# tensorlayer/HyperPose

Hardware: NVIDIA H100
Metric: frames/sec end-to-end (conv+PAF parse) OpenPose-COCO 368x656 (higher is better)
Workload: dtype f16 operands, f32 accumulate (conv); f32/f64 (parse)

## Files before the change

hyperpose_b200/capi.py:

```python
from __future__ import annotations

import ctypes as C
import os
import struct

import numpy as np

PKG = os.path.dirname(os.path.abspath(__file__))
LIB_PATH = os.path.join(PKG, "libhyperpose_b200.so")

N_PARTS, N_PAIRS = 18, 19
HP_OK, HP_ERR_ARG, HP_ERR_CAPACITY, HP_ERR_UNSUPPORTED, HP_ERR_CUDA, HP_ERR_BATCH = 0, -1, -2, -3, -4, -5

PART_DT = np.dtype({"names": ["has_value", "x", "y", "score"], "formats": ["<i4", "<f4", "<f4", "<f4"]})
HUMAN_DT = np.dtype([("parts", PART_DT, (N_PARTS,)), ("score", "<f4")])
PEAK_DT = np.dtype([("part_id", "<i4"), ("x", "<i4"), ("y", "<i4"), ("score", "<f4"), ("id", "<i4")])
CONN_DT = np.dtype([("cid1", "<i4"), ("cid2", "<i4"), ("score", "<f4")])
assert HUMAN_DT.itemsize == 292

EXPORTS = [
    "hp_last_error", "hp_device_count", "hp_version",
    "hp_paf_create", "hp_paf_destroy", "hp_paf_set_conf_thresh", "hp_paf_set_paf_thresh", "hp_paf_set_capacity",
    "hp_paf_process_host", "hp_paf_process_host_batched", "hp_paf_process_device", "hp_paf_fetch",
    "hp_paf_debug_peaks", "hp_paf_debug_connections", "hp_paf_launch_count", "hp_paf_copy_results_device", "hp_paf_debug_timing",
# ... 83 lines not shown
        return out[:n.value].copy()

    def process_batch(self, conf: np.ndarray, paf: np.ndarray, cap: int = 128):
        conf = np.ascontiguousarray(conf, np.float32)
        paf = np.ascontiguousarray(paf, np.float32)
        N = conf.shape[0]
        out = np.zeros((N, cap), HUMAN_DT)
        n = (C.c_int * N)()
        check(lib().hp_paf_process_host_batched(self._h, conf.ctypes.data, paf.ctypes.data, N, conf.shape[1], paf.shape[1],
                                                conf.shape[2], conf.shape[3], out.ctypes.data, cap, n))
        return [out[i, :n[i]].copy() for i in range(N)]

    def process_device(self, d_conf_ptr: int, d_paf_ptr: int, N, c_conf, c_paf, H, W, stream: int = 0):
        check(lib().hp_paf_process_device(self._h, d_conf_ptr, d_paf_ptr, N, c_conf, c_paf, H, W, stream))

    def fetch(self, N: int, cap: int = 128):
        out = np.zeros((N, cap), HUMAN_DT)
        n = (C.c_int * N)()
        check(lib().hp_paf_fetch(self._h, out.ctypes.data, cap, n, N))
        return [out[i, :n[i]].copy() for i in range(N)]

    def debug_peaks(self, frame: int = 0, cap: int = 1 << 16) -> np.ndarray:
        out = np.zeros(cap, PEAK_DT)
        n = C.c_int(0)
        check(lib().hp_paf_debug_peaks(self._h, frame, out.ctypes.data, cap, C.byref(n)))
        return out[:n.value].copy()

    def debug_connections(self, frame: int, pair_id: int, cap: int = 4096) -> np.ndarray:
        out = np.zeros(cap, CONN_DT)
        n = C.c_int(0)
        check(lib().hp_paf_debug_connections(self._h, frame, pair_id, out.ctypes.data, cap, C.byref(n)))
        return out[:n.value].copy()

    @property
    def launch_count(self) -> int:
        return int(lib().hp_paf_launch_count(self._h))

    def debug_timing(self, N: int):
        out = np.zeros(N * (N_PAIRS * 4 + 6), np.uint64)
        lib().hp_paf_debug_timing.argtypes = [C.c_void_p, C.c_void_p, C.c_int]
        check(lib().hp_paf_debug_timing(self._h, out.ctypes.data, N))
        return out[:N * N_PAIRS * 4].reshape(N, N_PAIRS, 4), out[N * N_PAIRS * 4:].reshape(N, 6)

    PLAN_FIELDS = ("generic", "rz_mode", "tab_staged", "stage_bytes", "limb_dyn_bytes", "fast_asm", "wide_tile_rows", "wide_tile_cols")

    def debug_plan(self) -> dict:
        out = np.zeros(len(self.PLAN_FIELDS), np.int32)
        lib().hp_paf_debug_plan.argtypes = [C.c_void_p, C.c_void_p, C.c_int]
        check(lib().hp_paf_debug_plan(self._h, out.ctypes.data, len(out)))
        return dict(zip(self.PLAN_FIELDS, (int(v) for v in out)))

    def copy_results_device(self, d_humans_ptr: int, d_counts_ptr: int, N: int, cap: int, stream: int = 0):
        check(lib().hp_paf_copy_results_device(self._h, d_humans_ptr, d_counts_ptr, N, cap, stream))


def handoff_stats() -> dict:
    L = lib()
    if not getattr(L, "_engine_bound", False):
        _bind_engine(L)
        L._engine_bound = True
    v = [C.c_longlong() for _ in range(4)]
    check(L.hp_handoff_stats(*[C.byref(x) for x in v]))
    return dict(zip(("published", "hits", "batch_parses", "misses"), [x.value for x in v]))


def handoff_enable(on: bool):
    L = lib()
    if not getattr(L, "_engine_bound", False):
        _bind_engine(L)
        L._engine_bound = True
    check(L.hp_handoff_enable(1 if on else 0))


EXPORTS += [
    "hp_engine_create", "hp_engine_destroy", "hp_engine_info", "hp_engine_infer_u8_host", "hp_engine_infer_u8_device",
    "hp_engine_infer_f32_host", "hp_engine_outputs", "hp_engine_read_outputs_host", "hp_engine_copy_outputs_device", "hp_engine_sync",
    "hp_engine_launch_count", "hp_engine_debug_read_buffer", "hp_engine_debug_write_buffer", "hp_engine_debug_run_ops",
    "hp_pose_run_u8_host", "hp_engine_stage_frame_u8", "hp_engine_infer_staged", "hp_engine_debug_read_frames", "hp_engine_set_output_override", "hp_engine_set_profiling", "hp_engine_get_profile",
    "hp_engine_read_outputs_frames", "hp_engine_head_type", "hp_handoff_enable", "hp_handoff_stats",
    "hp_pose_submit_u8_host", "hp_pose_collect", "hp_pose_stats", "hp_paf_prepare", "hp_paf_state", "hp_paf_copy_results_host_async",
    "hp_paf_grow_capacity", "hp_pool_create", "hp_pool_destroy", "hp_pool_size", "hp_pool_set_capacity", "hp_pool_run_u8_host",
    "hp_pool_set_output_override", "hp_pool_launch_count", "hp_default_device", "hp_handoff_device_of",
    "hp_engine_create_ex", "hp_engine_dtype", "hp_pose_submit_u8_device", "hp_engine_debug_op_kernel",
    "hp_engine_debug_op_epilogue", "hp_engine_debug_op_conv_epilogue", "hp_engine_debug_uses_pdl",
    "hp_engine_debug_read_buffer_raw", "hp_engine_debug_write_outputs",
    "hp_engine_calibrate_u8", "hp_pack_int8_calibrated",
    "hp_pose_submit_frames_u8_host", "hp_pose_submit_frames_u8_device", "hp_pose_submit_pifpaf_frames_u8_host",
    "hp_pose_submit_pifpaf_frames_u8_device", "hp_pose_debug_read_slot_frames",
    "hp_pose_submit_frames_yuv420_host", "hp_pose_submit_frames_yuv420_device", "hp_pose_submit_pifpaf_frames_yuv420_host",
    "hp_pose_submit_pifpaf_frames_yuv420_device", "hp_pose_submit_ppn_frames_yuv420_host", "hp_pose_submit_ppn_frames_yuv420_device",
    "hp_pose_submit_frames_interleaved_host", "hp_pose_submit_frames_interleaved_device", "hp_pose_submit_pifpaf_frames_interleaved_host",
    "hp_pose_submit_pifpaf_frames_interleaved_device", "hp_pose_submit_ppn_frames_interleaved_host",
    "hp_pose_submit_ppn_frames_interleaved_device",
] + [f"hp_pose_submit{head}_frames_{fmt}_rotated_{where}" for head in ("", "_pifpaf", "_ppn") for fmt in ("yuv420", "interleaved")
     for where in ("host", "device")]


class FrameU8(C.Structure):
    _fields_ = [("data", C.c_void_p), ("height", C.c_int32), ("width", C.c_int32)]


class FrameYUV420(C.Structure):
    _fields_ = [("y", C.c_void_p), ("u", C.c_void_p), ("v", C.c_void_p), ("height", C.c_int32), ("width", C.c_int32),
                ("pitch_y", C.c_int32), ("pitch_uv", C.c_int32), ("uv_step", C.c_int32)]


YUV420_LAYOUTS = {"nv12": lambda H, W: (H * W, H * W + 1, W, 2), "nv21": lambda H, W: (H * W + 1, H * W, W, 2),
                  "i420": lambda H, W: (H * W, H * W + H * W // 4, W // 2, 1), "yv12": lambda H, W: (H * W + H * W // 4, H * W, W // 2, 1)}


def yuv420_record(frame: np.ndarray, layout: str) -> FrameYUV420:
    H, W = frame.shape[0] * 2 // 3, frame.shape[1]
    u, v, pitch_uv, step = YUV420_LAYOUTS[layout](H, W)
    p = frame.ctypes.data
    return FrameYUV420(p, p + u, p + v, H, W, W, pitch_uv, step)


class FrameInterleaved(C.Structure):
    _fields_ = [("data", C.c_void_p), ("height", C.c_int32), ("width", C.c_int32), ("pitch", C.c_int32), ("format", C.c_int32)]


PIXEL_FORMATS = {"bgr": 0, "rgb": 1, "bgra": 2, "rgba": 3, "gray": 4, "yuyv": 5, "uyvy": 6, "yvyu": 7}
PIXEL_CHANNELS = {"bgr": 3, "rgb": 3, "bgra": 4, "rgba": 4, "gray": None, "yuyv": 2, "uyvy": 2, "yvyu": 2}


def interleaved_record(frame: np.ndarray, fmt: str) -> FrameInterleaved:
    return FrameInterleaved(frame.ctypes.data, frame.shape[0], frame.shape[1], frame.strides[0], PIXEL_FORMATS[fmt])


ROTATIONS = (0, 90, 180, 270)


def rotation_table(rotation, n: int):
    rots = None
    if isinstance(rotation, (int, np.integer)):
        rots = [rotation] * n
    elif isinstance(rotation, (list, tuple, np.ndarray)):
        rots = list(rotation)
    if rots is None or len(rots) != n:
        raise HyperposeError(HP_ERR_ARG, f"rotation {rotation!r}: expected one of {ROTATIONS} degrees, or one per frame ({n})")
    for i, r in enumerate(rots):
        if isinstance(r, (bool, np.bool_)) or not isinstance(r, (int, np.integer)) or int(r) not in ROTATIONS:
            raise HyperposeError(HP_ERR_ARG, f"frame {i}: rotation {r!r} is not one of {ROTATIONS} clockwise degrees")
    return (C.c_int32 * n)(*[int(r) for r in rots])


def _bind_engine(L):
    vp, ip = C.c_void_p, C.POINTER(C.c_int)
    L.hp_engine_create.argtypes = [C.POINTER(vp), vp, C.c_size_t, C.c_int, C.c_int, C.c_int, C.c_double, C.c_int, C.c_int]
    L.hp_engine_create_ex.argtypes = [C.POINTER(vp), vp, C.c_size_t, C.c_int, C.c_int, C.c_int, C.c_double, C.c_int, C.c_int, C.c_int]
    L.hp_engine_dtype.argtypes = [vp]
    L.hp_engine_destroy.argtypes = [vp]
    L.hp_engine_destroy.restype = None
    L.hp_engine_info.argtypes = [vp, ip, ip, ip, ip, ip, ip, ip, C.POINTER(C.c_double)]
    L.hp_engine_infer_u8_host.argtypes = [vp, vp, C.c_int]
    L.hp_engine_infer_u8_device.argtypes = [vp, vp, C.c_int, vp]
    L.hp_engine_infer_f32_host.argtypes = [vp, vp, C.c_int]
    L.hp_engine_outputs.argtypes = [vp, C.POINTER(vp), C.POINTER(vp), C.POINTER(vp)]
    L.hp_engine_read_outputs_host.argtypes = [vp, vp, vp, C.c_int]
    L.hp_engine_sync.argtypes = [vp]
    L.hp_engine_copy_outputs_device.argtypes = [vp, vp, vp, C.c_int, vp]
    L.hp_engine_launch_count.argtypes = [vp]
    L.hp_engine_launch_count.restype = C.c_longlong
    L.hp_engine_debug_read_buffer.argtypes = [vp, C.c_int, vp, C.c_int, ip, ip, ip]
    L.hp_engine_debug_write_buffer.argtypes = [vp, C.c_int, vp, C.c_int]
    L.hp_engine_debug_run_ops.argtypes = [vp, C.c_int, C.c_int, C.c_int]
    L.hp_engine_debug_op_kernel.argtypes = [vp, C.c_int, C.c_char_p, C.c_int]
    L.hp_engine_debug_op_epilogue.argtypes = [vp, C.c_int, ip]
    L.hp_engine_debug_op_conv_epilogue.argtypes = [vp, C.c_int, ip]
    L.hp_engine_debug_uses_pdl.argtypes = [vp, ip]
    L.hp_engine_debug_read_buffer_raw.argtypes = [vp, C.c_int, vp, C.c_int]
    L.hp_engine_debug_write_outputs.argtypes = [vp, vp, vp, C.c_int]
    L.hp_engine_calibrate_u8.argtypes = [vp, vp, C.c_int, vp, C.c_int]
    L.hp_pack_int8_calibrated.argtypes = [vp, C.c_size_t]
    L.hp_pose_run_u8_host.argtypes = [vp, vp, vp, C.c_int, vp, C.c_int, ip]
    L.hp_engine_stage_frame_u8.argtypes = [vp, C.c_int, vp, C.c_int, C.c_int, C.c_int]
    L.hp_engine_infer_staged.argtypes = [vp, C.c_int]
    L.hp_engine_debug_read_frames.argtypes = [vp, vp, C.c_int]
    L.hp_engine_set_output_override.argtypes = [vp, vp, vp]
    L.hp_engine_set_profiling.argtypes = [vp, C.c_int]
    L.hp_engine_get_profile.argtypes = [vp, vp, vp, vp, C.c_int, ip, C.POINTER(C.c_longlong)]
    L.hp_engine_read_outputs_frames.argtypes = [vp, C.POINTER(vp), C.POINTER(vp), C.c_int, C.c_int]
    L.hp_engine_head_type.argtypes = [vp]
    L.hp_handoff_enable.argtypes = [C.c_int]
    L.hp_handoff_stats.argtypes = [C.POINTER(C.c_longlong)] * 4
    L.hp_pose_submit_u8_host.argtypes = [vp, vp, vp, C.c_int, ip]
    L.hp_pose_submit_u8_device.argtypes = [vp, vp, vp, C.c_int, ip]
    L.hp_pose_collect.argtypes = [vp, C.c_int, vp, C.c_int, ip]
    for f in (L.hp_pose_submit_frames_u8_host, L.hp_pose_submit_frames_u8_device, L.hp_pose_submit_pifpaf_frames_u8_host,
              L.hp_pose_submit_pifpaf_frames_u8_device, L.hp_pose_submit_ppn_frames_u8_host, L.hp_pose_submit_ppn_frames_u8_device):
        f.argtypes = [vp, vp, C.POINTER(FrameU8), C.c_int, C.c_int, ip]
    for f in (L.hp_pose_submit_frames_yuv420_host, L.hp_pose_submit_frames_yuv420_device, L.hp_pose_submit_pifpaf_frames_yuv420_host,
              L.hp_pose_submit_pifpaf_frames_yuv420_device, L.hp_pose_submit_ppn_frames_yuv420_host, L.hp_pose_submit_ppn_frames_yuv420_device):
        f.argtypes = [vp, vp, C.POINTER(FrameYUV420), C.c_int, C.c_int, ip]
    for f in (L.hp_pose_submit_frames_interleaved_host, L.hp_pose_submit_frames_interleaved_device,
              L.hp_pose_submit_pifpaf_frames_interleaved_host, L.hp_pose_submit_pifpaf_frames_interleaved_device,
              L.hp_pose_submit_ppn_frames_interleaved_host, L.hp_pose_submit_ppn_frames_interleaved_device):
        f.argtypes = [vp, vp, C.POINTER(FrameInterleaved), C.c_int, C.c_int, ip]
    for head in ("", "_pifpaf", "_ppn"):
        for fmt, rec in (("yuv420", FrameYUV420), ("interleaved", FrameInterleaved)):
            for where in ("host", "device"):
                getattr(L, f"hp_pose_submit{head}_frames_{fmt}_rotated_{where}").argtypes = \
                    [vp, vp, C.POINTER(rec), C.POINTER(C.c_int32), C.c_int, C.c_int, ip]
    L.hp_pose_submit_ppn_u8_host.argtypes = [vp, vp, vp, C.c_int, ip]
    L.hp_pose_submit_ppn_u8_device.argtypes = [vp, vp, vp, C.c_int, ip]
    L.hp_pose_debug_read_slot_frames.argtypes = [vp, C.c_int, vp, C.c_int]
    L.hp_pose_stats.argtypes = [vp, C.POINTER(C.c_longlong), C.POINTER(C.c_longlong)]
    L.hp_pool_create.argtypes = [C.POINTER(vp), ip, C.c_int, vp, C.c_size_t, C.c_int, C.c_int, C.c_int, C.c_double, C.c_int, C.c_float, C.c_float]
    L.hp_pool_destroy.argtypes = [vp]
    L.hp_pool_destroy.restype = None
    L.hp_pool_size.argtypes = [vp]
    L.hp_pool_set_capacity.argtypes = [vp, C.c_int, C.c_int, C.c_int]
    L.hp_pool_run_u8_host.argtypes = [vp, vp, C.c_int, vp, C.c_int, ip]
    L.hp_pool_set_output_override.argtypes = [vp, C.POINTER(vp), C.POINTER(vp)]
    L.hp_pool_launch_count.argtypes = [vp]
    L.hp_pool_launch_count.restype = C.c_longlong
    L.hp_default_device.restype = C.c_int
    L.hp_handoff_device_of.argtypes = [vp]


class Engine:

    def __init__(self, pack: bytes, input_size, max_batch_size: int = 8, factor: float = 1.0 / 255, flip_rgb: bool = True,
                 device: int = 0, dtype: str = "f16"):
        L = lib()
        if not getattr(L, "_engine_bound", False):
            _bind_engine(L)
            L._engine_bound = True
        self._h = C.c_void_p()
        self._pack = pack
        self.dtype = dtype
        check(L.hp_engine_create_ex(C.byref(self._h), pack, len(pack), int(input_size[0]), int(input_size[1]), max_batch_size,
                                    factor, 1 if flip_rgb else 0, device, {"f16": 0, "tf32": 1, "int8": 2}[dtype]))
        v = [C.c_int() for _ in range(7)]
        fl = C.c_double()
        check(L.hp_engine_info(self._h, *[C.byref(x) for x in v], C.byref(fl)))
        (self.in_w, self.in_h, self.max_batch, self.c_conf, self.c_paf, self.out_h, self.out_w) = [x.value for x in v]
        self.flops_per_frame = fl.value

    def close(self):
        if getattr(self, "_h", None) and _lib is not None:
            _lib.hp_engine_destroy(self._h)
        self._h = None

    def __del__(self):
        try:
            self.close()
        except Exception:
            pass

    def max_batch_size(self):
        return self.max_batch
# ... 42 lines not shown
        return conf, paf

    def read_outputs_frames(self, n: int, publish: bool = False):
        if self.head_type == 1:
            sa, sb = (17, 5, self.out_h, self.out_w), (19, 9, self.out_h, self.out_w)
        else:
            sa, sb = (self.c_conf, self.out_h, self.out_w), (self.c_paf, self.out_h, self.out_w)
        a = [np.empty(sa, np.float32) for _ in range(n)]
        b = [np.empty(sb, np.float32) for _ in range(n)]
        pa = (C.c_void_p * n)(*[x.ctypes.data for x in a])
        pb = (C.c_void_p * n)(*[x.ctypes.data for x in b])
        check(lib().hp_engine_read_outputs_frames(self._h, pa, pb, n, 1 if publish else 0))
        return [[a[i], b[i]] for i in range(n)]

    @property
    def head_type(self) -> int:
        return int(lib().hp_engine_head_type(self._h))

    def device_outputs(self):
        a, b, s = C.c_void_p(), C.c_void_p(), C.c_void_p()
        check(lib().hp_engine_outputs(self._h, C.byref(a), C.byref(b), C.byref(s)))
        return a.value, b.value, (s.value or 0)

    def sync(self):
        check(lib().hp_engine_sync(self._h))

    def copy_outputs_device(self, d_conf_ptr: int, d_paf_ptr: int, n: int, stream: int = 0):
        check(lib().hp_engine_copy_outputs_device(self._h, d_conf_ptr, d_paf_ptr, n, stream))

    @property
    def launch_count(self) -> int:
        return int(lib().hp_engine_launch_count(self._h))

    def debug_read_buffer(self, buf: int, n: int, raw: bool = False) -> np.ndarray:
        H, W, Cc = C.c_int(), C.c_int(), C.c_int()
        check(lib().hp_engine_debug_read_buffer(self._h, buf, None, n, C.byref(H), C.byref(W), C.byref(Cc)))
        out = np.empty((n, H.value, W.value, Cc.value), self._elem)
        if raw:
            check(lib().hp_engine_debug_read_buffer_raw(self._h, buf, out.ctypes.data, n))
        else:
            check(lib().hp_engine_debug_read_buffer(self._h, buf, out.ctypes.data, n, C.byref(H), C.byref(W), C.byref(Cc)))
        return out

    def debug_write_outputs(self, conf: np.ndarray, paf: np.ndarray):
        conf, paf = np.ascontiguousarray(conf, np.float32), np.ascontiguousarray(paf, np.float32)
        assert conf.shape[0] == paf.shape[0]
        assert conf.shape[1:] == (self.c_conf, self.out_h, self.out_w) and paf.shape[1:] == (self.c_paf, self.out_h, self.out_w)
        check(lib().hp_engine_debug_write_outputs(self._h, conf.ctypes.data, paf.ctypes.data, conf.shape[0]))

    def debug_write_buffer(self, buf: int, arr: np.ndarray):
        arr = np.ascontiguousarray(arr, self._elem)
        check(lib().hp_engine_debug_write_buffer(self._h, buf, arr.ctypes.data, arr.shape[0]))

    @property
    def _elem(self):
        return {"f16": np.float16, "tf32": np.float32, "int8": np.int8}[self.dtype]

    def calibrate(self, frames: np.ndarray, absmax=None) -> np.ndarray:
        frames = np.ascontiguousarray(frames, np.uint8)
        assert frames.ndim == 4 and frames.shape[1:] == (self.in_h, self.in_w, 3), frames.shape
        n_buf = struct.unpack_from("<I", self._pack, 12)[0]
        out = np.zeros(n_buf, np.float32) if absmax is None else np.array(absmax, np.float32).reshape(-1).copy()
        check(lib().hp_engine_calibrate_u8(self._h, frames.ctypes.data, frames.shape[0], out.ctypes.data, out.size))
        return out

    def debug_run_ops(self, first: int, last: int, n: int):
        check(lib().hp_engine_debug_run_ops(self._h, first, last, n))

    def debug_op_kernel(self, op: int) -> str:
        buf = C.create_string_buffer(64)
        check(lib().hp_engine_debug_op_kernel(self._h, op, buf, len(buf)))
        return buf.value.decode()

    def debug_op_epilogue(self, op: int) -> str:
        v = C.c_int(0)
        check(lib().hp_engine_debug_op_epilogue(self._h, op, C.byref(v)))
        return "tma" if v.value else "reg"

    def debug_op_conv_epilogue(self, op: int) -> str:
        v = C.c_int(0)
        check(lib().hp_engine_debug_op_conv_epilogue(self._h, op, C.byref(v)))
        return "tma" if v.value else "reg"

    def debug_uses_pdl(self) -> bool:
        v = C.c_int(0)
        check(lib().hp_engine_debug_uses_pdl(self._h, C.byref(v)))
        return bool(v.value)

    def set_output_override(self, d_conf_ptr: int, d_paf_ptr: int):
        check(lib().hp_engine_set_output_override(self._h, d_conf_ptr, d_paf_ptr))

    def set_profiling(self, enable: bool):
        check(lib().hp_engine_set_profiling(self._h, 1 if enable else 0))

    def get_profile(self):
        cap = 1024
        ms = np.zeros(cap, np.float64); ty = np.zeros(cap, np.int32); fl = np.zeros(cap, np.float64)
        n, runs = C.c_int(), C.c_longlong()
        check(lib().hp_engine_get_profile(self._h, ms.ctypes.data, ty.ctypes.data, fl.ctypes.data, cap, C.byref(n), C.byref(runs)))
        return ms[:n.value], ty[:n.value], fl[:n.value], runs.value

    def run_pose(self, parser: "PafParser", frames: np.ndarray, cap: int = 128):
        frames = np.ascontiguousarray(frames, np.uint8)
        N = frames.shape[0]
        out = np.zeros((N, cap), HUMAN_DT)
        n = (C.c_int * N)()
        check(lib().hp_pose_run_u8_host(self._h, parser._h, frames.ctypes.data, N, out.ctypes.data, cap, n))
        return [out[i, :n[i]].copy() for i in range(N)]


    def submit_pose(self, parser: "PafParser", frames: np.ndarray) -> int:
        assert frames.dtype == np.uint8 and frames.flags["C_CONTIGUOUS"]
        t = C.c_int(-1)
        if isinstance(parser, PifPafParser):
            lib().hp_pose_submit_pifpaf_u8_host.argtypes = [C.c_void_p, C.c_void_p, C.c_void_p, C.c_int, C.POINTER(C.c_int)]
            check(lib().hp_pose_submit_pifpaf_u8_host(self._h, parser._h, frames.ctypes.data, frames.shape[0], C.byref(t)))
        elif isinstance(parser, PoseProposalParser):
            check(lib().hp_pose_submit_ppn_u8_host(self._h, parser._h, frames.ctypes.data, frames.shape[0], C.byref(t)))
        else:
            check(lib().hp_pose_submit_u8_host(self._h, parser._h, frames.ctypes.data, frames.shape[0], C.byref(t)))
        self._ticket_n = getattr(self, "_ticket_n", {})
        self._ticket_n[t.value] = frames.shape[0]
        return t.value

    def submit_pose_device(self, parser: "PafParser", d_frames_ptr: int, n: int) -> int:
        t = C.c_int(-1)
        if isinstance(parser, PifPafParser):
            lib().hp_pose_submit_pifpaf_u8_device.argtypes = [C.c_void_p, C.c_void_p, C.c_void_p, C.c_int, C.POINTER(C.c_int)]
            check(lib().hp_pose_submit_pifpaf_u8_device(self._h, parser._h, d_frames_ptr, n, C.byref(t)))
        elif isinstance(parser, PoseProposalParser):
            check(lib().hp_pose_submit_ppn_u8_device(self._h, parser._h, d_frames_ptr, n, C.byref(t)))
        else:
            check(lib().hp_pose_submit_u8_device(self._h, parser._h, d_frames_ptr, n, C.byref(t)))
        self._ticket_n = getattr(self, "_ticket_n", {})
        self._ticket_n[t.value] = n
        return t.value

    def _submit_frame_table(self, parser, table, keep_ratio, device: bool, fmt: str = "u8", rotation=None) -> int:
        t = C.c_int(-1)
        head = "_pifpaf" if isinstance(parser, PifPafParser) else "_ppn" if isinstance(parser, PoseProposalParser) else ""
        where = "device" if device else "host"
        if rotation is None:
            fn = getattr(lib(), f"hp_pose_submit{head}_frames_{fmt}_{where}")
            check(fn(self._h, parser._h, table, len(table), 1 if keep_ratio else 0, C.byref(t)))
        else:
            fn = getattr(lib(), f"hp_pose_submit{head}_frames_{fmt}_rotated_{where}")
            check(fn(self._h, parser._h, table, rotation, len(table), 1 if keep_ratio else 0, C.byref(t)))
        self._ticket_n = getattr(self, "_ticket_n", {})
        self._ticket_n[t.value] = len(table)
        return t.value

    def submit_pose_frames(self, parser, frames, keep_ratio: bool = False) -> int:
        for i, f in enumerate(frames):
            if not isinstance(f, np.ndarray) or f.dtype != np.uint8 or f.ndim != 3 or f.shape[2] != 3:
                raise HyperposeError(HP_ERR_ARG, f"frame {i}: expected a uint8 HWC array with 3 channels, got "
                                                 f"{getattr(f, 'dtype', type(f).__name__)} {getattr(f, 'shape', '')}")
        frames = [np.ascontiguousarray(f) for f in frames]
        table = (FrameU8 * len(frames))(*[FrameU8(f.ctypes.data, f.shape[0], f.shape[1]) for f in frames])
        t = self._submit_frame_table(parser, table, keep_ratio, device=False)
        self._ticket_frames = getattr(self, "_ticket_frames", {})
        self._ticket_frames[t] = frames
        return t

    def submit_pose_frames_device(self, parser, frames, keep_ratio: bool = False) -> int:
        table = (FrameU8 * len(frames))(*[FrameU8(int(p), int(h), int(w)) for p, h, w in frames])
        return self._submit_frame_table(parser, table, keep_ratio, device=True)
# ... 277 lines not shown
```

hyperpose_b200/csrc/conv_wgmma.cuh:

```cuda
#pragma once
#include <cuda.h>
#include <cuda_fp16.h>
#include <cuda_runtime.h>
#include <stdint.h>

#include <type_traits>

namespace hpb {

constexpr int CONV_BLOCK_M = 128;
constexpr int CONV_BLOCK_K = 64;
constexpr int TF32_BLOCK_K = 32;
constexpr int CONV_MAX_STAGES = 8;
constexpr int CONV_THREADS = 384;
constexpr int CONV_A_BYTES = CONV_BLOCK_M * 128;
constexpr size_t CONV_SMEM_LIMIT = 227 * 1024;

enum ConvOutMode : int {
    OUT_F16_NHWC = 0,
    OUT_F32_NCHW_SPLIT = 1,
};

struct ConvParams {
    int Nb, H, W;
// ... 679 lines not shown
                        if (p.post_w) {
                            const int pc = t.g * p.cout_g + t.n0 + c;
                            const float2 x = __half22float2(h2);
                            float y0 = fmaf(x.x, __ldg(p.post_w + pc), 0.f) + __ldg(p.post_b + pc);
                            float y1 = two ? fmaf(x.y, __ldg(p.post_w + pc + 1), 0.f) + __ldg(p.post_b + pc + 1) : 0.f;
                            y0 = y0 > 0.f ? y0 : y0 * __ldg(p.post_a + pc);
                            if (two) y1 = y1 > 0.f ? y1 : y1 * __ldg(p.post_a + pc + 1);
                            h2 = __floats2half2_rn(y0, y1);
                        }
                        __half* o = (__half*)p.out + pix * p.out_ld + och + c;
                        if (two && pair_ok) *(__half2*)o = h2;
                        else { o[0] = __low2half(h2); if (two) o[1] = __high2half(h2); }
                    } else {
                        float* o = (float*)p.out + pix * p.out_ld + och + c;
                        const float y0 = ptx::round_tf32(a0), y1 = ptx::round_tf32(a1);
                        if (two && pair_ok) *(float2*)o = make_float2(y0, y1);
                        else { o[0] = y0; if (two) o[1] = y1; }
                    }
                } else {
#pragma unroll
                    for (int e = 0; e < 2; ++e) {
                        if (e == 1 && !two) break;
                        const int ch = t.n0 + c + e;
                        const float y = e ? a1 : a0;
                        if (ch < p.split) {
                            ((float*)p.out)[(((size_t)q.n * p.split + ch) * p.H + q.h) * p.W + q.w] = y;
                        } else {
                            const int c2 = ch - p.split, n2 = p.cout_g - p.split;
                            ((float*)p.out2)[(((size_t)q.n * n2 + c2) * p.H + q.h) * p.W + q.w] = y;
                        }
                    }
                }
            }
        }
    }
    if (tma && (threadIdx.x & 127) == 0) ptx::bulk_wait<0>();
}

constexpr size_t CONV_SMEM_FIXED = 1024  + 2 * CONV_MAX_STAGES * 8;
inline size_t conv_smem_bytes(int BN, int stages, bool tma_store)
{
    return CONV_SMEM_FIXED + (size_t)stages * (CONV_A_BYTES + BN * 128) + (tma_store ? 2 * (size_t)BN * 128 : 0);
}
inline int conv_pick_stages(int BN, bool tma_store)
{
    int s = CONV_MAX_STAGES;
    while (s > 2 && conv_smem_bytes(BN, s, tma_store) > CONV_SMEM_LIMIT) --s;
    return s;
}

constexpr int HALO_TH = 16, HALO_TW = 8;

constexpr int HALO_WIDE_PRODUCER_REGS = 40, HALO_WIDE_CONSUMER_REGS = 232;


#ifdef HPB_HALO_PHASES
enum { HALO_PH_TOTAL, HALO_PH_A_WAIT, HALO_PH_B_WAIT, HALO_PH_MMA_WAIT, HALO_PH_EPILOGUE, HALO_PH_TURN_WAIT, HALO_PH_STAGE_WAIT, HALO_PH_COUNT };
__device__ unsigned long long g_halo_phases[HALO_PH_COUNT];
#define HALO_PH_MARK(t) const long long t = clock64()
#define HALO_TIMED(i, ...) do { const long long t0_ = clock64(); __VA_ARGS__; ph[i] += clock64() - t0_; } while (0)
#define HALO_PH_ADD(i, t) (ph[i] += clock64() - (t))
#define HALO_PH_PARAM , long long (&ph)[HALO_PH_COUNT]
#define HALO_PH_ARG , ph
#else
#define HALO_PH_MARK(t) do {} while (0)
#define HALO_TIMED(i, ...) do { __VA_ARGS__; } while (0)
#define HALO_PH_ADD(i, t) do {} while (0)
#define HALO_PH_PARAM
#define HALO_PH_ARG
#endif

struct HaloParams {
    int Nb, H, W;
    int R, S, groups, cin_g;
    int cout_g, cout_g_pad;
    int in_ch_off;
    int tiles_x, tiles_y;
    int box_bytes;
    int num_stages;
    const float* bias; const float* alpha;
    __half* out; int out_ld, out_ch_off;
    int tma_store;
    int stage_bytes;
};

enum class HaloItem { Narrow, Wide, PingPong };
struct HaloShape {
    int tiles;
    int blocks;
    int box_slots;
    int slot_warps;
    int stage_slots;
    bool move_regs;
};
__host__ __device__ constexpr HaloShape halo_shape(HaloItem it, int BN)
{
    return it == HaloItem::Wide       ? HaloShape{ 2, 2, 2, 8, 0, true }
           : it == HaloItem::PingPong ? HaloShape{ 1, 2, 4, 4, BN == 64 ? 2 : 1, true }
                                      : HaloShape{ 1, 1, 2, 8, 1, false };
}
inline int halo_stage_bytes(int BN, HaloItem it) { return halo_shape(it, BN).stage_slots * BN * 128; }

namespace ptx {
__device__ __forceinline__ uint64_t make_sw128_kmajor_desc_at(uint32_t smem_addr, uint32_t sbo)
{
    uint64_t d = 0;
    d |= (uint64_t)((smem_addr & 0x3ffffu) >> 4);
    d |= (uint64_t)1 << 16;
    d |= (uint64_t)((sbo >> 4) & 0x3fffu) << 32;
    d |= (uint64_t)1 << 62;
    return d;
}
template <uint32_t N> __device__ __forceinline__ void setmaxnreg_dec() { asm volatile("setmaxnreg.dec.sync.aligned.u32 %0;" ::"n"(N)); }
template <uint32_t N> __device__ __forceinline__ void setmaxnreg_inc() { asm volatile("setmaxnreg.inc.sync.aligned.u32 %0;" ::"n"(N)); }
__device__ __forceinline__ void st_shared_u32(uint32_t addr, uint32_t v) { asm volatile("st.shared.b32 [%0], %1;" ::"r"(addr), "r"(v) : "memory"); }
__device__ __forceinline__ void tma_store_4d(const CUtensorMap* m, uint32_t src, int c0, int c1, int c2, int c3)
{
    asm volatile("cp.async.bulk.tensor.4d.global.shared::cta.bulk_group [%0, {%2, %3, %4, %5}], [%1];"
                 ::"l"(m), "r"(src), "r"(c0), "r"(c1), "r"(c2), "r"(c3) : "memory");
}
}

template <int BN, bool kPool, int kBlocks>
__device__ __forceinline__ void halo_epilogue(const float (&acc)[kBlocks][BN / 2], const HaloParams& p, int n, int y0, int x0, int g, int n0,
                                              int row_base, int warp, int lane)
{
    const int col0 = 2 * (lane & 3);
    const int tx = lane >> 2;
    const float* bias = p.bias + g * p.cout_g_pad + n0;
    const float* alpha = p.alpha + g * p.cout_g_pad + n0;
    const int och = p.out_ch_off + g * p.cout_g + n0;
    const bool pair_ok = ((och | p.out_ld) & 1) == 0;
    if constexpr (kPool) {
#pragma unroll
        for (int m = 0; m < kBlocks; ++m) {
            const int ty0 = row_base + m * 8 + (warp & 3) * 2;
            const float (&acc0)[BN / 2] = acc[m];
            const int py = (y0 + ty0) >> 1, px = (x0 + tx) >> 1;
            const bool store = (tx & 1) == 0 && py < (p.H >> 1) && px < (p.W >> 1);
            __half* o = p.out + (((size_t)n * (p.H >> 1) + py) * (p.W >> 1) + px) * p.out_ld + och;
#pragma unroll
            for (int j = 0; j < BN / 8; ++j) {
                float v0 = fmaxf(acc0[4 * j], acc0[4 * j + 2]), v1 = fmaxf(acc0[4 * j + 1], acc0[4 * j + 3]);
                v0 = fmaxf(v0, __shfl_xor_sync(0xffffffffu, v0, 4));
                v1 = fmaxf(v1, __shfl_xor_sync(0xffffffffu, v1, 4));
                const int c = 8 * j + col0;
                if (!store) continue;
                float a0 = v0 + __ldg(bias + c), a1 = v1 + __ldg(bias + c + 1);
                a0 = a0 > 0.f ? a0 : a0 * __ldg(alpha + c);
                a1 = a1 > 0.f ? a1 : a1 * __ldg(alpha + c + 1);
                const __half2 h2 = __floats2half2_rn(a0, a1);
                if (pair_ok) *(__half2*)(o + c) = h2;
                else { o[c] = __low2half(h2); o[c + 1] = __high2half(h2); }
            }
        }
    } else {
        const int n_valid = min(BN, p.cout_g - n0);
#pragma unroll
        for (int m = 0; m < kBlocks; ++m) {
            const int ty0 = row_base + m * 8 + (warp & 3) * 2;
#pragma unroll
            for (int h = 0; h < 2; ++h) {
                const int oy = y0 + ty0 + h, ox = x0 + tx;
                if (oy >= p.H || ox >= p.W) continue;
                __half* o = p.out + (((size_t)n * p.H + oy) * p.W + ox) * p.out_ld + och;
#pragma unroll
                for (int j = 0; j < BN / 8; ++j) {
                    const int c = 8 * j + col0;
                    if (c >= n_valid) break;
                    float a0 = acc[m][4 * j + 2 * h] + __ldg(bias + c), a1 = acc[m][4 * j + 2 * h + 1] + __ldg(bias + c + 1);
                    a0 = a0 > 0.f ? a0 : a0 * __ldg(alpha + c);
                    a1 = a1 > 0.f ? a1 : a1 * __ldg(alpha + c + 1);
                    const __half2 h2 = __floats2half2_rn(a0, a1);
                    const bool two = c + 1 < n_valid;
                    if (two && pair_ok) *(__half2*)(o + c) = h2;
                    else { o[c] = __low2half(h2); if (two) o[c + 1] = __high2half(h2); }
                }
            }
        }
    }
}

template <int BN, bool kPool, int kBlocks, int kSlots, bool kWait>
__device__ __forceinline__ void halo_epilogue_tma(const float (&acc)[kBlocks][BN / 2], const HaloParams& p, const CUtensorMap* tmap_o, uint32_t stage,
                                                  int n, int y0, int x0, int g, int n0, int row_base, int warp, int lane, bool leader HALO_PH_PARAM)
{
    static_assert(BN == 64 || BN == 128, "one TMA box per 64-channel slice, at most two");
    constexpr int kSliceBytes = (kPool ? 16 : 64) * 128;
    constexpr int kSlotBytes = BN / 64 * kSliceBytes;
    const int col0 = 2 * (lane & 3);
    const float* bias = p.bias + g * p.cout_g_pad + n0;
    const float* alpha = p.alpha + g * p.cout_g_pad + n0;
    const int och = p.out_ch_off + g * p.cout_g + n0;
    const int bar_id = warp >> 2;
#pragma unroll
    for (int m = 0; m < kBlocks; ++m) {
        const uint32_t slot = stage + (uint32_t)((m % kSlots) * kSlotBytes);
        HALO_PH_MARK(t_wait);
        if (kWait && leader) ptx::bulk_wait_read<kSlots - 1>();
        ptx::named_barrier_sync(bar_id, 128);
#ifdef HPB_HALO_PHASES
        { const long long d = clock64() - t_wait; ph[HALO_PH_STAGE_WAIT] += d; ph[HALO_PH_EPILOGUE] -= d; }
#endif
        const int ty0 = row_base + m * 8;
        if constexpr (kPool) {
            const int q = (warp & 3) * 4 + (lane >> 3);
            const bool store = ((lane >> 2) & 1) == 0;
#pragma unroll
            for (int j = 0; j < BN / 8; ++j) {
                float v0 = fmaxf(acc[m][4 * j], acc[m][4 * j + 2]), v1 = fmaxf(acc[m][4 * j + 1], acc[m][4 * j + 3]);
                v0 = fmaxf(v0, __shfl_xor_sync(0xffffffffu, v0, 4));
                v1 = fmaxf(v1, __shfl_xor_sync(0xffffffffu, v1, 4));
                if (!store) continue;
                const int c = 8 * j + col0;
                const float2 b = __ldg((const float2*)(bias + c)), a = __ldg((const float2*)(alpha + c));
                float a0 = v0 + b.x, a1 = v1 + b.y;
                a0 = a0 > 0.f ? a0 : a0 * a.x;
                a1 = a1 > 0.f ? a1 : a1 * a.y;
                ptx::st_shared_u32(slot + (uint32_t)((j >> 3) * kSliceBytes + q * 128 + (((j & 7) ^ (q & 7)) << 4) + (lane & 3) * 4),
                                   ptx::half2_bits(__floats2half2_rn(a0, a1)));
            }
        } else {
            const int r = lane & 7, i = lane >> 3;
#pragma unroll
            for (int jb = 0; jb < BN / 32; ++jb) {
                float2 b[4], a[4];
#pragma unroll
                for (int k = 0; k < 4; ++k) {
                    const int c = 8 * (4 * jb + k) + col0;
                    b[k] = __ldg((const float2*)(bias + c));
                    a[k] = __ldg((const float2*)(alpha + c));
                }
#pragma unroll
                for (int h = 0; h < 2; ++h) {
                    uint32_t v[4];
#pragma unroll
                    for (int k = 0; k < 4; ++k) {
                        float a0 = acc[m][4 * (4 * jb + k) + 2 * h] + b[k].x, a1 = acc[m][4 * (4 * jb + k) + 2 * h + 1] + b[k].y;
                        a0 = a0 > 0.f ? a0 : a0 * a[k].x;
                        a1 = a1 > 0.f ? a1 : a1 * a[k].y;
                        v[k] = ptx::half2_bits(__floats2half2_rn(a0, a1));
                    }
                    const int j = 4 * jb + i, row = (warp & 3) * 16 + 8 * h + r;
                    ptx::stmatrix_x4(slot + (uint32_t)((j >> 3) * kSliceBytes + row * 128 + (((j & 7) ^ r) << 4)), v[0], v[1], v[2], v[3]);
                }
            }
        }
        ptx::fence_proxy_async();
        ptx::named_barrier_sync(bar_id, 128);
        if (leader) {
            const int x = kPool ? x0 >> 1 : x0, y = kPool ? (y0 + ty0) >> 1 : y0 + ty0;
            ptx::tma_store_4d(tmap_o, slot, och, x, y, n);
            if (BN == 128 && n0 + 64 < p.cout_g)
                ptx::tma_store_4d(tmap_o, slot + (uint32_t)kSliceBytes, och + 64, x, y, n);
            ptx::bulk_commit();
        }
    }
}

template <int BN, int kBlocks>
__device__ __forceinline__ void halo_kstep(float (&acc)[kBlocks][BN / 2], uint32_t abase, int r, int s, int BW, uint32_t sbo, const uint8_t* s_b,
                                           uint64_t* b_full, RingPos b, int c_or_tap HALO_PH_PARAM)
{
    uint64_t da[kBlocks];
#pragma unroll
    for (int m = 0; m < kBlocks; ++m) da[m] = ptx::make_sw128_kmajor_desc_at(abase + (uint32_t)(((m * 8 + r) * BW + s) * 128), sbo);
    const uint64_t db = ptx::make_sw128_kmajor_desc(ptx::smem_u32(s_b + (size_t)b.slot * BN * 128));
    HALO_TIMED(HALO_PH_B_WAIT, ptx::mbar_wait(ptx::smem_u32(b_full + b.slot), b.phase));
#pragma unroll
    for (int m = 0; m < kBlocks; ++m) ptx::fence_acc(acc[m]);
    ptx::wgmma_fence();
#pragma unroll
    for (int k = 0; k < 4; ++k)
#pragma unroll
        for (int m = 0; m < kBlocks; ++m)
            ptx::wgmma<__half, BN>(acc[m], da[m] + (uint64_t)(k * 2), db + (uint64_t)(k * 2), (c_or_tap | k) != 0 ? 1u : 0u);
    ptx::wgmma_commit();
#pragma unroll
    for (int m = 0; m < kBlocks; ++m) ptx::fence_acc(acc[m]);
}

template <int BN, bool kPool, HaloItem kItem>
__device__ __forceinline__ void halo_store(const float (&acc)[halo_shape(kItem, BN).blocks][BN / 2], const HaloParams& p, const CUtensorMap* tmap_o,
                                           bool tma, uint32_t stage, int n, int y0, int x0, int g, int n0, int row_base, int warp, int lane,
                                           bool leader HALO_PH_PARAM)
{
    constexpr HaloShape kShape = halo_shape(kItem, BN);
    if constexpr (BN % 64 == 0) {
        if (tma) {
            if constexpr (kItem != HaloItem::Wide)
                halo_epilogue_tma<BN, kPool, kShape.blocks, kShape.stage_slots, true>(acc, p, tmap_o, stage, n, y0, x0, g, n0, row_base, warp, lane,
                                                                                     leader HALO_PH_ARG);
            else if (p.box_bytes >= kShape.blocks * BN * 128)
                halo_epilogue_tma<BN, kPool, kShape.blocks, kShape.blocks, false>(acc, p, tmap_o, stage, n, y0, x0, g, n0, row_base, warp, lane,
                                                                                 leader HALO_PH_ARG);
            else
                halo_epilogue_tma<BN, kPool, kShape.blocks, 1, true>(acc, p, tmap_o, stage, n, y0, x0, g, n0, row_base, warp, lane, leader HALO_PH_ARG);
            return;
        }
    }
    halo_epilogue<BN, kPool, kShape.blocks>(acc, p, n, y0, x0, g, n0, row_base, warp, lane);
}

template <int BN, bool kPool, HaloItem kItem>
__global__ void __launch_bounds__(CONV_THREADS, 1)
conv_halo_kernel(const __grid_constant__ CUtensorMap tmap_x, const __grid_constant__ CUtensorMap tmap_b, const __grid_constant__ CUtensorMap tmap_o,
                 const HaloParams p)
{
    static_assert(!(kItem == HaloItem::Wide && kPool), "the pooled epilogue pairs pixel rows of one m64 block; it has no wide form");
    static_assert(kItem != HaloItem::PingPong || BN == 64 || BN == 128, "the ping-pong item is built for the VGG trunk's widths, BN = 64 and 128");
    constexpr HaloShape kShape = halo_shape(kItem, BN);
    constexpr int B_BYTES = BN * 128;
    constexpr bool kTmaForm = BN % 64 == 0;
    extern __shared__ uint8_t smem_raw[];
    ptx::pdl_launch_dependents();
    uint8_t* smem = (uint8_t*)(((uintptr_t)smem_raw + 1023) & ~(uintptr_t)1023);
    uint8_t* s_box = smem;
    uint8_t* s_b = s_box + (size_t)kShape.box_slots * kShape.tiles * p.box_bytes;
    uint8_t* s_stage = s_b + (size_t)p.num_stages * B_BYTES;
    uint64_t* a_full = (uint64_t*)(s_stage + 2 * (size_t)p.stage_bytes);
    uint64_t* a_empty = a_full + kShape.box_slots;
    uint64_t* b_full = a_empty + kShape.box_slots;
    uint64_t* b_empty = b_full + CONV_MAX_STAGES;
    uint64_t* turn = b_empty + CONV_MAX_STAGES;

    const int wg = threadIdx.x >> 7, warp = threadIdx.x >> 5, lane = threadIdx.x & 31;
    const int n_tiles_g = p.cout_g_pad / BN;
    const int nt_total = p.groups * n_tiles_g;
    const int sp_per_img = p.tiles_x * p.tiles_y;
    const int total_items = (p.Nb * sp_per_img + kShape.tiles - 1) / kShape.tiles * nt_total;
    const int chunks = p.cin_g / CONV_BLOCK_K;
    const int taps = p.R * p.S;
    const int BW = HALO_TW + p.S - 1, BH = HALO_TH + p.R - 1;

    if (threadIdx.x == 0) {
        ptx::prefetch_tmap(&tmap_x);
        ptx::prefetch_tmap(&tmap_b);
        if (kTmaForm && p.tma_store) ptx::prefetch_tmap(&tmap_o);
        for (int i = 0; i < kShape.box_slots; ++i) {
            ptx::mbar_init(ptx::smem_u32(a_full + i), 1);
            ptx::mbar_init(ptx::smem_u32(a_empty + i), kShape.slot_warps);
        }
        for (int i = 0; i < p.num_stages; ++i) {
            ptx::mbar_init(ptx::smem_u32(b_full + i), 1);
            ptx::mbar_init(ptx::smem_u32(b_empty + i), kShape.slot_warps);
        }
        if constexpr (kItem == HaloItem::PingPong) {
            ptx::mbar_init(ptx::smem_u32(turn), 4);
            ptx::mbar_init(ptx::smem_u32(turn + 1), 4);
        }
        ptx::fence_barrier_init();
    }
    __syncthreads();
    ptx::pdl_wait();

    auto decode = [&](int item, int& sp, int& g, int& n0) {
        const int nt = item % nt_total;
        sp = item / nt_total * kShape.tiles;
        g = nt / n_tiles_g;
        n0 = (nt - g * n_tiles_g) * BN;
    };
    auto tile_pos = [&](int sp, int& n, int& y0, int& x0) {
        n = sp / sp_per_img;
        const int t = sp - n * sp_per_img;
        const int ty = t / p.tiles_x;
        y0 = ty * HALO_TH;
        x0 = (t - ty * p.tiles_x) * HALO_TW;
    };

#ifdef HPB_HALO_PHASES
    long long ph[HALO_PH_COUNT] = {};
    HALO_PH_MARK(t_start);
#endif
    RingPos a, b;
    if (wg == 0) {
        if constexpr (kShape.move_regs) ptx::setmaxnreg_dec<HALO_WIDE_PRODUCER_REGS>();
        if (warp == 0 && ptx::elect_one()) {
            const int pad_h = p.R / 2, pad_w = p.S / 2;
            for (int item = blockIdx.x; item < total_items; item += gridDim.x) {
                int sp, g, n0;
                decode(item, sp, g, n0);
                for (int c = 0; c < chunks; ++c) {
                    ptx::mbar_wait(ptx::smem_u32(a_empty + a.slot), a.phase ^ 1);
                    const uint32_t fa = ptx::smem_u32(a_full + a.slot);
                    ptx::mbar_expect_tx(fa, (uint32_t)(kShape.tiles * BH * BW * 128));
#pragma unroll
                    for (int t = 0; t < kShape.tiles; ++t) {
                        int n, y0, x0;
                        tile_pos(sp + t, n, y0, x0);
                        ptx::tma_load_4d(ptx::smem_u32(s_box + (size_t)(a.slot * kShape.tiles + t) * p.box_bytes), &tmap_x, fa,
                                         p.in_ch_off + g * p.cin_g + c * CONV_BLOCK_K, x0 - pad_w, y0 - pad_h, n);
                    }
                    a.step(kShape.box_slots);
                    for (int tap = 0; tap < taps; ++tap) {
                        ptx::mbar_wait(ptx::smem_u32(b_empty + b.slot), b.phase ^ 1);
                        const uint32_t fb = ptx::smem_u32(b_full + b.slot);
                        ptx::mbar_expect_tx(fb, (uint32_t)B_BYTES);
                        ptx::tma_load_2d(ptx::smem_u32(s_b + (size_t)b.slot * B_BYTES), &tmap_b, fb, tap * p.cin_g + c * CONV_BLOCK_K, g * p.cout_g_pad + n0);
                        b.step(p.num_stages);
                    }
                }
            }
        }
        return;
    }

    if constexpr (kShape.move_regs) ptx::setmaxnreg_inc<HALO_WIDE_CONSUMER_REGS>();
    const int half = wg - 1;
    const uint32_t sbo = (uint32_t)BW * 128u;
    const bool tma = kTmaForm && p.tma_store;
    const bool leader = (threadIdx.x & 127) == 0;
    const uint32_t stage = ptx::smem_u32(s_stage + (size_t)half * p.stage_bytes);
    float acc[kShape.blocks][BN / 2];
    if constexpr (kItem == HaloItem::PingPong) {
        const int item_stages = chunks * taps;
        if (half) {
            a.advance(chunks, kShape.box_slots);
            b.advance(item_stages, p.num_stages);
        }
        for (int j = half, item = blockIdx.x + half * gridDim.x; item < total_items; j += 2, item += 2 * gridDim.x) {
            int sp, g, n0;
            decode(item, sp, g, n0);
            if (j > 0) HALO_TIMED(HALO_PH_TURN_WAIT, ptx::mbar_wait(ptx::smem_u32(turn + half), (uint32_t)((j - 1) >> 1) & 1u));
            int prev_st = 0, prev_bs = 0;
            for (int c = 0; c < chunks; ++c) {
                HALO_TIMED(HALO_PH_A_WAIT, ptx::mbar_wait(ptx::smem_u32(a_full + a.slot), a.phase));
                const uint32_t abase = ptx::smem_u32(s_box + (size_t)a.slot * p.box_bytes);
                for (int tap = 0; tap < taps; ++tap) {
                    const int r = tap / p.S, s = tap - r * p.S;
                    halo_kstep<BN, kShape.blocks>(acc, abase, r, s, BW, sbo, s_b, b_full, b, c | tap HALO_PH_ARG);
                    if ((c | tap) != 0) {
                        HALO_TIMED(HALO_PH_MMA_WAIT, ptx::wgmma_wait<1>());
                        if (lane == 0) {
                            ptx::mbar_arrive(ptx::smem_u32(b_empty + prev_st));
                            if (tap == 0) ptx::mbar_arrive(ptx::smem_u32(a_empty + prev_bs));
                        }
                    }
                    prev_st = b.slot;
                    b.step(p.num_stages);
                }
                prev_bs = a.slot;
                a.step(kShape.box_slots);
            }
            if (lane == 0) ptx::mbar_arrive(ptx::smem_u32(turn + (half ^ 1)));
            HALO_TIMED(HALO_PH_MMA_WAIT, ptx::wgmma_wait<0>());
#pragma unroll
            for (int m = 0; m < kShape.blocks; ++m) ptx::fence_acc(acc[m]);
            if (lane == 0) {
                ptx::mbar_arrive(ptx::smem_u32(b_empty + prev_st));
                ptx::mbar_arrive(ptx::smem_u32(a_empty + prev_bs));
            }
            a.advance(chunks, kShape.box_slots);
            b.advance(item_stages, p.num_stages);
            HALO_PH_MARK(t_epi);
            int n, y0, x0;
            tile_pos(sp, n, y0, x0);
            halo_store<BN, kPool, kItem>(acc, p, &tmap_o, tma, stage, n, y0, x0, g, n0, 0, warp, lane, leader HALO_PH_ARG);
            HALO_PH_ADD(HALO_PH_EPILOGUE, t_epi);
        }
    } else {
        const int box = kItem == HaloItem::Wide ? half : 0;
        const int row_base = kItem == HaloItem::Wide ? 0 : half * 8;
        int held = -1;
        for (int item = blockIdx.x; item < total_items; item += gridDim.x) {
            int sp, g, n0;
            decode(item, sp, g, n0);
            for (int c = 0; c < chunks; ++c) {
                HALO_TIMED(HALO_PH_A_WAIT, ptx::mbar_wait(ptx::smem_u32(a_full + a.slot), a.phase));
                const uint32_t abase = ptx::smem_u32(s_box + (size_t)(a.slot * kShape.tiles + box) * p.box_bytes) + (uint32_t)(row_base * BW * 128);
                int prev = 0;
                for (int tap = 0; tap < taps; ++tap) {
                    const int r = tap / p.S, s = tap - r * p.S;
                    halo_kstep<BN, kShape.blocks>(acc, abase, r, s, BW, sbo, s_b, b_full, b, c | tap HALO_PH_ARG);
                    if (tap > 0) {
                        HALO_TIMED(HALO_PH_MMA_WAIT, ptx::wgmma_wait<1>());
                        if (lane == 0) ptx::mbar_arrive(ptx::smem_u32(b_empty + prev));
                    }
                    if (kItem == HaloItem::Wide && held >= 0 && tap == taps / 2) {
                        HALO_TIMED(HALO_PH_STAGE_WAIT, ptx::bulk_wait_read<0>());
                        ptx::mbar_arrive(ptx::smem_u32(a_empty + held));
                        held = -1;
                    }
                    prev = b.slot;
                    b.step(p.num_stages);
                }
                HALO_TIMED(HALO_PH_MMA_WAIT, ptx::wgmma_wait<0>());
#pragma unroll
                for (int m = 0; m < kShape.blocks; ++m) ptx::fence_acc(acc[m]);
                if (lane == 0) {
                    ptx::mbar_arrive(ptx::smem_u32(b_empty + prev));
                    if (kItem == HaloItem::Wide && tma && leader && c == chunks - 1) held = a.slot;
                    else ptx::mbar_arrive(ptx::smem_u32(a_empty + a.slot));
                }
                a.step(kShape.box_slots);
            }

            HALO_PH_MARK(t_epi);
            int n, y0, x0;
            tile_pos(sp + box, n, y0, x0);
            if (kItem == HaloItem::Wide && n >= p.Nb) {
                if (held >= 0) { ptx::mbar_arrive(ptx::smem_u32(a_empty + held)); held = -1; }
                continue;
            }
            const int last = (a.slot + kShape.box_slots - 1) % kShape.box_slots;
            const uint32_t dst = kItem == HaloItem::Wide ? ptx::smem_u32(s_box + (size_t)(last * kShape.tiles + box) * p.box_bytes) : stage;
            halo_store<BN, kPool, kItem>(acc, p, &tmap_o, tma, dst, n, y0, x0, g, n0, row_base, warp, lane, leader HALO_PH_ARG);
            HALO_PH_ADD(HALO_PH_EPILOGUE, t_epi);
        }
    }
    if (tma && leader) ptx::bulk_wait<0>();
#ifdef HPB_HALO_PHASES
    HALO_PH_ADD(HALO_PH_TOTAL, t_start);
    if ((threadIdx.x & 127) == 0)
        for (int i = 0; i < HALO_PH_COUNT; ++i) atomicAdd(g_halo_phases + i, (unsigned long long)ph[i]);
#endif
}

inline int halo_box_bytes(int R, int S) { return ((HALO_TH + R - 1) * (HALO_TW + S - 1) * 128 + 1023) & ~1023; }
inline size_t conv_halo_smem_bytes(int R, int S, int BN, int stages, HaloItem it, bool tma_store)
{
    const HaloShape sh = halo_shape(it, BN);
    return 1024 + (size_t)sh.box_slots * sh.tiles * halo_box_bytes(R, S) + (size_t)stages * BN * 128 +
           (tma_store ? 2 * (size_t)halo_stage_bytes(BN, it) : 0) + (2 * sh.box_slots + 2 * CONV_MAX_STAGES + 2) * 8;
}
inline int conv_halo_pick_stages(int R, int S, int BN, HaloItem it, bool tma_store)
{
    int s = CONV_MAX_STAGES;
    while (s > 2 && conv_halo_smem_bytes(R, S, BN, s, it, tma_store) > CONV_SMEM_LIMIT) --s;
    return s;
}

}
```

hyperpose_b200/csrc/engine.cu:

```cuda
#include <cuda.h>
#include <cuda_fp16.h>
#include <cuda_runtime.h>
#include <math.h>
#include <stdint.h>
#include <stdlib.h>
#include <string.h>

#include <algorithm>
#include <memory>
#include <string>
#include <vector>

#include "../../include/hyperpose_b200.h"
#include "common.h"
#include "conv_wgmma.cuh"
#include "helpers_tf32_int8.cuh"
#include "handoff.h"
#include "pair_math.cuh"
#include "pack_format.h"

namespace {
using namespace hpb;


// ... 626 lines not shown
}
int elem_bytes(int dtype) { return dtype == HP_DTYPE_TF32 ? 4 : dtype == HP_DTYPE_INT8 ? 1 : 2; }

int make_tmap_act_im2col(CUtensorMap* m, const void* base, int N, int H, int W, int C, int R, int S, int dtype)
{
    const int es = elem_bytes(dtype);
    const auto enc = (PFN_encodeIm2col)driver_entry_point("cuTensorMapEncodeIm2col");
    if (!enc) { set_error("cuTensorMapEncodeIm2col entry point not available"); return HP_ERR_CUDA; }
    cuuint64_t dims[4] = { (cuuint64_t)C, (cuuint64_t)W, (cuuint64_t)H, (cuuint64_t)N };
    cuuint64_t strides[3] = { (cuuint64_t)C * es, (cuuint64_t)W * C * es, (cuuint64_t)H * W * C * es };
    const int pad_w = S / 2, pad_h = R / 2;
    int lower[2] = { -pad_w, -pad_h };
    int upper[2] = { pad_w - (S - 1), pad_h - (R - 1) };
    cuuint32_t estr[4] = { 1, 1, 1, 1 };
    CUresult r = enc(m, tmap_type(dtype), 4, (void*)base, dims, strides, lower, upper, 128 / es, (cuuint32_t)CONV_BLOCK_M, estr,
                     CU_TENSOR_MAP_INTERLEAVE_NONE, CU_TENSOR_MAP_SWIZZLE_128B, CU_TENSOR_MAP_L2_PROMOTION_L2_256B, CU_TENSOR_MAP_FLOAT_OOB_FILL_NONE);
    if (r != CUDA_SUCCESS) { set_error("cuTensorMapEncodeIm2col failed: %d (N=%d H=%d W=%d C=%d R=%d S=%d)", (int)r, N, H, W, C, R, S); return HP_ERR_CUDA; }
    return HP_OK;
}
int make_tmap_wgt(CUtensorMap* m, const void* base, int rows, int K, int BN, int dtype)
{
    const int es = elem_bytes(dtype);
    const auto enc = (PFN_encodeTiled)driver_entry_point("cuTensorMapEncodeTiled");
    if (!enc) { set_error("cuTensorMapEncodeTiled entry point not available"); return HP_ERR_CUDA; }
    cuuint64_t dims[2] = { (cuuint64_t)K, (cuuint64_t)rows };
    cuuint64_t strides[1] = { (cuuint64_t)K * es };
    cuuint32_t box[2] = { (cuuint32_t)(128 / es), (cuuint32_t)BN };
    cuuint32_t estr[2] = { 1, 1 };
    CUresult r = enc(m, tmap_type(dtype), 2, (void*)base, dims, strides, box, estr, CU_TENSOR_MAP_INTERLEAVE_NONE,
                     CU_TENSOR_MAP_SWIZZLE_128B, CU_TENSOR_MAP_L2_PROMOTION_L2_256B, CU_TENSOR_MAP_FLOAT_OOB_FILL_NONE);
    if (r != CUDA_SUCCESS) { set_error("cuTensorMapEncodeTiled(weights) failed: %d (rows=%d K=%d BN=%d)", (int)r, rows, K, BN); return HP_ERR_CUDA; }
    return HP_OK;
}

int make_tmap_act_box(CUtensorMap* m, const __half* base, int N, int H, int W, int C, int ld, int box_w, int box_h, CUtensorMapSwizzle swizzle)
{
    const auto enc = (PFN_encodeTiled)driver_entry_point("cuTensorMapEncodeTiled");
    if (!enc) { set_error("cuTensorMapEncodeTiled entry point not available"); return HP_ERR_CUDA; }
    cuuint64_t dims[4] = { (cuuint64_t)C, (cuuint64_t)W, (cuuint64_t)H, (cuuint64_t)N };
    cuuint64_t strides[3] = { (cuuint64_t)ld * 2, (cuuint64_t)W * ld * 2, (cuuint64_t)H * W * ld * 2 };
    cuuint32_t box[4] = { 64, (cuuint32_t)box_w, (cuuint32_t)box_h, 1 };
    cuuint32_t estr[4] = { 1, 1, 1, 1 };
    CUresult r = enc(m, CU_TENSOR_MAP_DATA_TYPE_FLOAT16, 4, (void*)base, dims, strides, box, estr, CU_TENSOR_MAP_INTERLEAVE_NONE,
                     swizzle, CU_TENSOR_MAP_L2_PROMOTION_L2_256B, CU_TENSOR_MAP_FLOAT_OOB_FILL_NONE);
    if (r != CUDA_SUCCESS) { set_error("cuTensorMapEncodeTiled(box) failed: %d (N=%d H=%d W=%d C=%d ld=%d box %dx%d)", (int)r, N, H, W, C, ld, box_w, box_h); return HP_ERR_CUDA; }
    return HP_OK;
}

int make_tmap_pixel_rows(CUtensorMap* m, const __half* base, long pixels, int C, int ld)
{
    const auto enc = (PFN_encodeTiled)driver_entry_point("cuTensorMapEncodeTiled");
    if (!enc) { set_error("cuTensorMapEncodeTiled entry point not available"); return HP_ERR_CUDA; }
    cuuint64_t dims[2] = { (cuuint64_t)C, (cuuint64_t)pixels };
    cuuint64_t strides[1] = { (cuuint64_t)ld * 2 };
    cuuint32_t box[2] = { 64, 64 };
    cuuint32_t estr[2] = { 1, 1 };
    CUresult r = enc(m, CU_TENSOR_MAP_DATA_TYPE_FLOAT16, 2, (void*)base, dims, strides, box, estr, CU_TENSOR_MAP_INTERLEAVE_NONE,
                     CU_TENSOR_MAP_SWIZZLE_128B, CU_TENSOR_MAP_L2_PROMOTION_L2_256B, CU_TENSOR_MAP_FLOAT_OOB_FILL_NONE);
    if (r != CUDA_SUCCESS) { set_error("cuTensorMapEncodeTiled(pixel rows) failed: %d (pixels=%ld C=%d ld=%d)", (int)r, pixels, C, ld); return HP_ERR_CUDA; }
    return HP_OK;
}

int round_up(int a, int b) { return (a + b - 1) / b * b; }

int pick_bn(int cout_g)
{
    if (cout_g <= 16) return 16;
    if (cout_g <= 32) return 32;
    if (cout_g <= 48) return 48;
    if (cout_g <= 64) return 64;
    if (cout_g <= 96) return 96;
    if (cout_g <= 128) return 128;
    int best = 128;
    for (int bn : { 96, 64 })
        if (round_up(cout_g, bn) < round_up(cout_g, best)) best = bn;
    return best;
}

struct ConvPlan {
    ConvParams prm;
    CUtensorMap tmap_a, tmap_b;
    CUtensorMap tmap_x;
    CUtensorMap tmap_o;
    void* d_w = nullptr;
    bool monotone_act = false;
    HaloParams hp;
    HaloItem halo_item = HaloItem::Narrow;
    bool halo_pool = false;
    float* d_bias = nullptr;
    float* d_alpha = nullptr;
    float* d_mul = nullptr;
    size_t smem = 0;
    double flops_per_frame = 0;
};

enum class Launch : uint8_t {
    None,
    Im2col,
    StemOrIm2col,
    Conv,
    ConvStem,
    Halo,
    DwTma,
    DwTmaPair,
    DwCol,
    DwStrip,
    MaxPool,
    Heads,
    PpnHead,
    Im2colC4,
    DwC4,
    MaxPoolC4,
};

int kernels_launched(Launch k, bool u8_input)
{
    switch (k) {
    case Launch::None: return 0;
    case Launch::StemOrIm2col: return u8_input ? 0 : 1;
    case Launch::Heads: return 2;
    default: return 1;
    }
}

bool reads_buffer(const PackOp& q, uint32_t b)
{
    if (q.type == OP_IM2COL3) return false;
    return q.in_buf == b || (((q.type == OP_CONV && q.res_mode) || q.type == OP_PIFPAF_HEAD) && q.res_buf == b);
}

struct EngOp {
    Launch launch = Launch::None;
    PackOp po;
    ConvPlan plan;
    float* d_dw = nullptr;
    CUtensorMap tmap_dw;
    int dwt_wbo = 0, dwt_hb = 0, dwt_tiles_x = 0, dwt_tiles_y = 0, dwt_stages = 0;
    size_t dwt_smem = 0;
};

struct EngOptions {
    enum { HALO_AUTO, HALO_NONE, HALO_ALL } halo = HALO_AUTO;
    bool halo_wide = true;
    bool halo_tma_store = true;
    bool conv_tma_store = true;
    bool stem3 = true;
    bool pool_fuse = true;
    bool dw1_fuse = true;
    bool dw_pair = true;
    bool dw_tma = true;
    int pifpaf_reserve_sms = 0;
};

inline int same_pad_before(int in, int k, int stride)
{
    const int out = (in + stride - 1) / stride;
    const int total = std::max((out - 1) * stride + k - in, 0);
    return total / 2;
}

inline int dw_dilation(const PackOp& po) { return po.dilation ? (int)po.dilation : 1; }

struct EngBuffer {
    bool fused_away = false;
    int channels = 0, down = 0, H = 0, W = 0;
    __half* d = nullptr;
};

}

struct hp_engine {
    int device = 0;
    int dtype = 0;
    std::vector<float> act_scale;
    int in_h = 0, in_w = 0, max_batch = 0;
    double factor = 1.0 / 255;
    int flip_rgb = 1;
    int num_sms = 132;
    EngOptions opt;
    PackHeader hdr;
    std::vector<EngBuffer> bufs;
    std::vector<EngOp> ops;
    int step_kernels = 0;
    float* d_conf = nullptr;
    float* d_paf = nullptr;
    int out_h = 0, out_w = 0;
    int ppn_K = 0, ppn_E = 0, ppn_nh = 0, ppn_nw = 0;
    uint8_t* d_frames = nullptr;
    float* d_input_f32 = nullptr;
    uint8_t* pin_frames = nullptr;
    cudaStream_t stream = nullptr;
    long long launches = 0;
    double flops_per_frame = 0;
    int last_N = 0;
    uint8_t* d_src = nullptr; size_t d_src_bytes = 0;
    uint8_t* pin_src = nullptr; size_t pin_src_bytes = 0;
    FrameDesc* d_stage_desc = nullptr; FrameDesc* pin_stage_desc = nullptr;
    const float* override_conf = nullptr;
    const float* override_paf = nullptr;
    bool profiling = false;
    static constexpr int EV_DEPTH = 4;
    std::vector<cudaEvent_t> ev;
    std::vector<double> op_ms_sum;
    long long profiled_runs = 0;
    long long ev_head = 0, ev_tail = 0;
    float* pin_out = nullptr; size_t pin_out_floats = 0;
    std::shared_ptr<hpb::handoff::Batch> ho_ring[hpb::handoff::HANDOFF_RING];
    int ho_pos = 0;
    const uint8_t* cur_frames = nullptr;
    bool stage_synced = false;
    struct PoseSlot {
        uint8_t* d_frames = nullptr;
        uint8_t* pin_frames = nullptr;
        uint8_t* d_src = nullptr; size_t d_src_bytes = 0;
        uint8_t* pin_src = nullptr; size_t pin_src_bytes = 0;
        FrameDesc* d_desc = nullptr; FrameDesc* pin_desc = nullptr;
        YuvFrameDesc* d_ydesc = nullptr; YuvFrameDesc* pin_ydesc = nullptr;
        InterleavedFrameDesc* d_idesc = nullptr; InterleavedFrameDesc* pin_idesc = nullptr;
        hp_human* pin_humans = nullptr; size_t pin_humans_n = 0;
        int* pin_counts = nullptr; size_t pin_counts_n = 0;
        cudaEvent_t h2d_done = nullptr, done = nullptr;
        bool busy = false;
        int N = 0, hcap = 0;
        hp_paf* parser = nullptr;
        hp_ppn* ppn = nullptr;
        hp_pifpaf* decoder = nullptr;
        cudaEvent_t conv_done = nullptr;
        cudaGraphExec_t graph = nullptr;
        float key_f[3] = { 0, 0, 0 }; int key_i[6] = { 0, 0, 0, 0, 0, 0 }; int key_N = 0; const void* key_parser = nullptr;
        const void* key_ovr[2] = { nullptr, nullptr };
    } slots[2];
    int next_slot = 0;
    bool use_pdl = false;
    int reserve_sms = 0;
    cudaEvent_t heads_wait = nullptr;
    cudaStream_t copy_stream = nullptr;
    bool graphs_ok = true;
    long long graph_launches = 0, graph_captures = 0;
};

namespace {

inline float tf32_round(float x)
{
    uint32_t u;
    memcpy(&u, &x, 4);
    if ((u & 0x7f800000u) != 0x7f800000u) u = (u + 0x1000u) & 0xffffe000u;
    memcpy(&x, &u, 4);
    return x;
}

bool halo_tma_store_ok(const HaloParams& h, int BN)
{
    return BN % 64 == 0 && h.out_ld % 8 == 0 && h.out_ch_off % 8 == 0 && (h.groups * h.cout_g) % 8 == 0 &&
           (h.groups == 1 || h.cout_g % BN == 0);
}

int set_halo_item(const hp_engine* e, EngOp& op, HaloItem item, bool pool)
{
    HaloParams& h = op.plan.hp;
    const int BN = op.plan.prm.BN;
    h.tma_store = e->opt.halo_tma_store && halo_tma_store_ok(h, BN);
    h.stage_bytes = h.tma_store ? halo_stage_bytes(BN, item) : 0;
    h.num_stages = conv_halo_pick_stages(h.R, h.S, BN, item, h.tma_store);
    op.plan.smem = conv_halo_smem_bytes(h.R, h.S, BN, h.num_stages, item, h.tma_store);
    op.plan.halo_item = item;
    op.plan.halo_pool = pool;
    op.launch = Launch::Halo;
    if (!h.tma_store) return HP_OK;
    const int oh = pool ? h.H / 2 : h.H, ow = pool ? h.W / 2 : h.W, box = pool ? HALO_TW / 2 : HALO_TW;
    return make_tmap_act_box(&op.plan.tmap_o, h.out, e->max_batch, oh, ow, h.out_ch_off + h.groups * h.cout_g, h.out_ld, box, box,
                             CU_TENSOR_MAP_SWIZZLE_128B);
}

int set_conv_tma_store(const hp_engine* e, EngOp& op)
{
    ConvParams& p = op.plan.prm;
    p.tma_store = e->opt.conv_tma_store && e->dtype == HP_DTYPE_F16 && p.out_mode == OUT_F16_NHWC && (p.BN == 64 || p.BN == 128) &&
                  p.out_ld % 8 == 0 && p.out_ch_off % 8 == 0 && (p.groups * p.cout_g) % 8 == 0 && (p.groups == 1 || p.cout_g % p.BN == 0);
    p.num_stages = conv_pick_stages(p.BN, p.tma_store);
    op.plan.smem = conv_smem_bytes(p.BN, p.num_stages, p.tma_store);
    if (!p.tma_store) return HP_OK;
    return make_tmap_pixel_rows(&op.plan.tmap_o, (const __half*)p.out, (long)e->max_batch * p.H * p.W, p.out_ch_off + p.groups * p.cout_g, p.out_ld);
}

bool halo_wide_faster(int R, long wide_items, int sms)
{
    return R == 7 && wide_items >= sms;
}

bool halo_pp_exists(int R, int BN) { return R == 3 && (BN == 64 || BN == 128); }
bool halo_pp_faster(int chunks, bool pooled, long items, int sms) { return (chunks >= 4 || pooled) && items >= 2L * sms; }

HaloItem pick_halo_item(const hp_engine* e, const EngOp& op, bool pooled)
{
    const HaloParams& h = op.plan.hp;
    const int BN = op.plan.prm.BN, sms = e->num_sms - e->reserve_sms;
    const long tiles = (long)h.Nb * h.tiles_x * h.tiles_y, n_tiles = (long)h.groups * (h.cout_g_pad / BN);
    const bool all = e->opt.halo == EngOptions::HALO_ALL;
    if (!e->opt.halo_wide) return HaloItem::Narrow;
    if (!pooled && BN == 128 && conv_halo_pick_stages(h.R, h.S, BN, HaloItem::Wide, false) >= 3 && (all || halo_wide_faster(h.R, (tiles + 1) / 2 * n_tiles, sms)))
        return HaloItem::Wide;
    if (halo_pp_exists(h.R, BN) && (all || halo_pp_faster(h.cin_g / CONV_BLOCK_K, pooled, tiles * n_tiles, sms))) return HaloItem::PingPong;
    return HaloItem::Narrow;
}

int build_conv_plan(hp_engine* e, EngOp& op, const float* blob)
{
    const PackOp& po = op.po;
    ConvPlan& pl = op.plan;
    const bool tf32 = e->dtype == HP_DTYPE_TF32, i8 = e->dtype == HP_DTYPE_INT8;
    const int chunk = tf32 ? 32 : i8 ? 128 : 64;
    const size_t es = (size_t)elem_bytes(e->dtype);
    const EngBuffer& ib = e->bufs[po.in_buf];
    const int G = (int)po.groups, R = (int)po.R, S = (int)po.S, cin_g = (int)po.cin_g, cout_g = (int)po.cout_g;
    const bool im2col = po.im2col_input != 0;
    if (im2col && (G != 1 || R * S * cin_g > ib.channels)) { set_error("engine: bad im2col conv"); return HP_ERR_ARG; }
    if (!im2col && G > 1 && cin_g % (i8 ? 16 : chunk) != 0) { set_error("engine: grouped conv needs cin_g %% %d == 0 (got %d)", i8 ? 16 : chunk, cin_g); return HP_ERR_UNSUPPORTED; }
    const int eR = im2col ? 1 : R, eS = im2col ? 1 : S;
    const int ecin = im2col ? round_up(R * S * cin_g, chunk) : round_up(cin_g, chunk);
    const int reads = i8 ? (im2col ? R * S * cin_g : G * cin_g) : G * ecin;
    if ((int)po.in_ch_off + reads > ib.channels) {
        set_error("engine: conv reads channels [%d,%d) of a %d-channel buffer", po.in_ch_off, po.in_ch_off + reads, ib.channels);
        return HP_ERR_ARG;
    }
    if (i8 && (long long)R * S * cin_g * 127 * 127 > 0x7fffffffLL) {
        set_error("engine: INT8 conv op %d sums %d products per output (%dx%dx%d); the s32 accumulator is exact up to %d", (int)(&op - e->ops.data()), R * S * cin_g,
                  R, S, cin_g, 0x7fffffff / (127 * 127));
        return HP_ERR_UNSUPPORTED;
    }
    if (i8 && ib.channels % 16) {
        set_error("engine: INT8 conv op %d reads buffer %u of %d channels (needs a multiple of 16)", (int)(&op - e->ops.data()), po.in_buf, ib.channels);
        return HP_ERR_ARG;
    }
    const int BN = pick_bn(cout_g);
    const int cout_pad = round_up(cout_g, BN);
    const int K = eR * eS * ecin;
    std::vector<float> w((size_t)G * cout_pad * K, 0.f), bias((size_t)G * cout_pad, 0.f), alpha((size_t)G * cout_pad, 0.f);
    const float* W = blob + po.w_off;
    for (int g = 0; g < G; ++g)
        for (int o = 0; o < cout_g; ++o) {
            bias[(size_t)g * cout_pad + o] = blob[po.b_off + (size_t)g * cout_g + o];
            alpha[(size_t)g * cout_pad + o] = blob[po.a_off + (size_t)g * cout_g + o];
            for (int c = 0; c < cin_g; ++c)
                for (int r = 0; r < R; ++r)
                    for (int s = 0; s < S; ++s) {
                        const float v = W[((((size_t)g * cout_g + o) * cin_g + c) * R + r) * S + s];
                        const size_t k = im2col ? (size_t)((r * S + s) * cin_g + c) : ((size_t)(r * S + s) * ecin + c);
                        w[((size_t)g * cout_pad + o) * K + k] = tf32 ? tf32_round(v) : v;
                    }
        }
    std::vector<__half> wh;
    if (!tf32 && !i8) {
        wh.resize(w.size());
        for (size_t i = 0; i < w.size(); ++i) wh[i] = __float2half_rn(w[i]);
    }
    std::vector<int8_t> wq;
    std::vector<float> mul;
    if (i8) {
        wq.assign(w.size(), 0);
        mul.assign(bias.size(), 0.f);
        const float s_in = e->act_scale[po.in_buf];
        for (size_t row = 0; row < (size_t)G * cout_pad; ++row) {
            if ((int)(row % cout_pad) >= cout_g) continue;
            const float* wr = w.data() + row * K;
            float amax = 0.f;
            for (int k = 0; k < K; ++k) amax = std::max(amax, fabsf(wr[k]));
            const float sw = amax > 0.f ? amax / 127.0f : 1.0f;
            for (int k = 0; k < K; ++k) wq[row * K + k] = (int8_t)std::min(127.0f, std::max(-127.0f, nearbyintf(wr[k] / sw)));
            mul[row] = s_in * sw;
        }
        HP_CUDA_TRY(cudaMalloc(&pl.d_mul, mul.size() * sizeof(float)));
        HP_CUDA_TRY(cudaMemcpy(pl.d_mul, mul.data(), mul.size() * sizeof(float), cudaMemcpyHostToDevice));
    }
    HP_CUDA_TRY(cudaMalloc(&pl.d_w, w.size() * es));
    HP_CUDA_TRY(cudaMalloc(&pl.d_bias, bias.size() * sizeof(float)));
    HP_CUDA_TRY(cudaMalloc(&pl.d_alpha, alpha.size() * sizeof(float)));
    HP_CUDA_TRY(cudaMemcpy(pl.d_w, tf32 ? (const void*)w.data() : i8 ? (const void*)wq.data() : (const void*)wh.data(), w.size() * es, cudaMemcpyHostToDevice));
    HP_CUDA_TRY(cudaMemcpy(pl.d_bias, bias.data(), bias.size() * sizeof(float), cudaMemcpyHostToDevice));
    HP_CUDA_TRY(cudaMemcpy(pl.d_alpha, alpha.data(), alpha.size() * sizeof(float), cudaMemcpyHostToDevice));

    ConvParams& p = pl.prm;
    memset(&p, 0, sizeof(p));
    p.Nb = e->max_batch; p.H = ib.H; p.W = ib.W;
    p.R = eR; p.S = eS; p.groups = G; p.cin_g = ecin;
    p.cout_g = cout_g; p.cout_g_pad = cout_pad; p.BN = BN;
    p.m_tiles = (int)(((size_t)e->max_batch * p.H * p.W + CONV_BLOCK_M - 1) / CONV_BLOCK_M);
    p.in_ch_off = (int)po.in_ch_off;
    p.num_stages = conv_pick_stages(BN, false);
// ... 9 lines not shown
            set_error("engine: output conv op %d reads a %dx%d buffer but the outputs are %dx%d conf/paf planes (head_type %u)",
                      (int)(&op - e->ops.data()), ib.H, ib.W, e->out_h, e->out_w, e->hdr.head_type);
            return HP_ERR_ARG;
        }
    } else {
        const EngBuffer& ob = e->bufs[po.out_buf];
        if (ob.H != ib.H || ob.W != ib.W || (int)po.out_ch_off + G * cout_g > ob.channels) { set_error("engine: conv output buffer mismatch"); return HP_ERR_ARG; }
        p.out = ob.d; p.out_ld = ob.channels; p.out_ch_off = (int)po.out_ch_off;
        if (i8) p.out_inv_scale = 1.0f / e->act_scale[po.out_buf];
    }
    if (i8) { p.mul = pl.d_mul; p.in_g_stride = cin_g; }
    if (po.res_mode) {
        if (po.out_mode != OUT_F16_NHWC || po.res_buf >= e->bufs.size()) { set_error("engine: bad residual"); return HP_ERR_ARG; }
        const EngBuffer& rb = e->bufs[po.res_buf];
        if (rb.H != ib.H || rb.W != ib.W || (int)po.res_ch_off + G * cout_g > rb.channels || po.res_ch_off % 8 || cout_g % 16) { set_error("engine: residual buffer mismatch"); return HP_ERR_ARG; }
        p.res = rb.d; p.res_ld = rb.channels; p.res_ch_off = (int)po.res_ch_off; p.res_mode = (int)po.res_mode;
        if (i8) p.res_scale = e->act_scale[po.res_buf];
    }
    int rc = make_tmap_act_im2col(&pl.tmap_a, ib.d, e->max_batch, ib.H, ib.W, ib.channels, eR, eS, e->dtype);
    if (rc) return rc;
    rc = make_tmap_wgt(&pl.tmap_b, pl.d_w, G * cout_pad, K, BN, e->dtype);
    if (rc) return rc;
    pl.smem = conv_smem_bytes(BN, p.num_stages, false);
    pl.flops_per_frame = 2.0 * ib.H * ib.W * (double)G * cout_g * cin_g * R * S;
    op.launch = Launch::Conv;
    if (e->dtype != HP_DTYPE_F16) return HP_OK;
    pl.monotone_act = true;
    for (float a : alpha) if (!(a >= 0.f)) { pl.monotone_act = false; break; }
    const int ty = (ib.H + HALO_TH - 1) / HALO_TH, tx = (ib.W + HALO_TW - 1) / HALO_TW;
    const double waste = (double)ty * HALO_TH * tx * HALO_TW / ((double)ib.H * ib.W) - 1.0;
    const bool shape_ok = !im2col && eR == eS && (eR == 3 || eR == 5 || eR == 7) && !po.res_mode && po.out_mode == OUT_F16_NHWC;
    const bool rounds = (long)p.m_tiles * G * (cout_pad / BN) > e->num_sms - e->reserve_sms;
    const bool faster = (eR == 3 && waste <= 0.06) || (rounds && ecin >= 2 * CONV_BLOCK_K && waste <= 0.25);
    const bool want = e->opt.halo == EngOptions::HALO_AUTO ? faster : e->opt.halo == EngOptions::HALO_ALL;
    if (shape_ok && want) {
        const EngBuffer& ob = e->bufs[po.out_buf];
        HaloParams& h = pl.hp;
        memset(&h, 0, sizeof(h));
        h.Nb = e->max_batch; h.H = ib.H; h.W = ib.W; h.R = eR; h.S = eS; h.groups = G; h.cin_g = ecin;
        h.cout_g = cout_g; h.cout_g_pad = cout_pad; h.in_ch_off = (int)po.in_ch_off;
        h.tiles_x = tx; h.tiles_y = ty;
        h.box_bytes = halo_box_bytes(eR, eS);
        h.bias = pl.d_bias; h.alpha = pl.d_alpha;
        h.out = ob.d; h.out_ld = ob.channels; h.out_ch_off = (int)po.out_ch_off;
        rc = make_tmap_act_box(&pl.tmap_x, ib.d, e->max_batch, ib.H, ib.W, ib.channels, ib.channels, HALO_TW + eS - 1, HALO_TH + eR - 1, CU_TENSOR_MAP_SWIZZLE_128B);
        if (rc) return rc;
        rc = set_halo_item(e, op, pick_halo_item(e, op, false), false);
        if (rc) return rc;
    }
    return HP_OK;
}

thread_local bool tl_use_pdl = false;
static inline cudaLaunchConfig_t pdl_config(int grid, int block, size_t smem, cudaStream_t st, cudaLaunchAttribute* at)
{
    cudaLaunchConfig_t cfg = {};
    cfg.gridDim = dim3((unsigned)grid); cfg.blockDim = dim3((unsigned)block); cfg.dynamicSmemBytes = smem; cfg.stream = st;
    at[0].id = cudaLaunchAttributeProgrammaticStreamSerialization;
    at[0].val.programmaticStreamSerializationAllowed = 1;
    cfg.attrs = at; cfg.numAttrs = tl_use_pdl ? 1 : 0;
    return cfg;
}
template <typename... KArgs, typename... Args>
static inline void launch_pdl(void (*kernel)(KArgs...), int grid, int block, size_t smem, cudaStream_t st, Args&&... args)
{
    cudaLaunchAttribute at[1];
    const cudaLaunchConfig_t cfg = pdl_config(grid, block, smem, st, at);
    cudaLaunchKernelEx(&cfg, kernel, std::forward<Args>(args)...);
}

template <typename T, bool kRes, int kStemR = 0>
const void* conv_kernel_bn(int BN)
{
    switch (BN) {
    case 16: return (const void*)conv_wgmma_kernel<T, 16, kRes, kStemR>;
    case 32: return (const void*)conv_wgmma_kernel<T, 32, kRes, kStemR>;
    case 48: return (const void*)conv_wgmma_kernel<T, 48, kRes, kStemR>;
    case 64: return (const void*)conv_wgmma_kernel<T, 64, kRes, kStemR>;
    case 96: return (const void*)conv_wgmma_kernel<T, 96, kRes, kStemR>;
    case 128: return (const void*)conv_wgmma_kernel<T, 128, kRes, kStemR>;
    }
    return nullptr;
}
const void* halo_kernel(int BN, HaloItem item, bool pool)
{
    using I = HaloItem;
    if (item == I::Wide) return BN == 128 && !pool ? (const void*)conv_halo_kernel<128, false, I::Wide> : nullptr;
    if (item == I::PingPong) {
        if (BN == 64) return pool ? (const void*)conv_halo_kernel<64, true, I::PingPong> : (const void*)conv_halo_kernel<64, false, I::PingPong>;
        if (BN == 128) return pool ? (const void*)conv_halo_kernel<128, true, I::PingPong> : (const void*)conv_halo_kernel<128, false, I::PingPong>;
        return nullptr;
    }
    switch (BN) {
    case 16: return pool ? (const void*)conv_halo_kernel<16, true, I::Narrow> : (const void*)conv_halo_kernel<16, false, I::Narrow>;
    case 32: return pool ? (const void*)conv_halo_kernel<32, true, I::Narrow> : (const void*)conv_halo_kernel<32, false, I::Narrow>;
    case 48: return pool ? (const void*)conv_halo_kernel<48, true, I::Narrow> : (const void*)conv_halo_kernel<48, false, I::Narrow>;
    case 64: return pool ? (const void*)conv_halo_kernel<64, true, I::Narrow> : (const void*)conv_halo_kernel<64, false, I::Narrow>;
    case 96: return pool ? (const void*)conv_halo_kernel<96, true, I::Narrow> : (const void*)conv_halo_kernel<96, false, I::Narrow>;
    case 128: return pool ? (const void*)conv_halo_kernel<128, true, I::Narrow> : (const void*)conv_halo_kernel<128, false, I::Narrow>;
    }
    return nullptr;
}
const void* conv_kernel(int dtype, bool res, int BN, int stem_R = 0)
{
    if (stem_R == 3) return conv_kernel_bn<__half, false, 3>(BN);
    if (stem_R == 7) return conv_kernel_bn<__half, false, 7>(BN);
    if (dtype == HP_DTYPE_TF32) return res ? conv_kernel_bn<float, true>(BN) : conv_kernel_bn<float, false>(BN);
    if (dtype == HP_DTYPE_INT8) return res ? conv_kernel_bn<int8_t, true>(BN) : conv_kernel_bn<int8_t, false>(BN);
    return res ? conv_kernel_bn<__half, true>(BN) : conv_kernel_bn<__half, false>(BN);
}

void launch_dw_tma(hp_engine* e, const EngOp& op, const EngOp* pair, int N, cudaStream_t st)
{
    const PackOp& po = op.po;
    const EngBuffer& ib = e->bufs[po.in_buf];
    const EngBuffer& ob = e->bufs[po.out_buf];
    DwTmaParams p;
    p.out0 = ob.d + po.out_ch_off;
    p.out1 = pair ? e->bufs[pair->po.out_buf].d + pair->po.out_ch_off : nullptr;
    p.out_ld = ob.channels;
    p.w0 = op.d_dw; p.w1 = pair ? pair->d_dw : nullptr;
    p.H = ib.H; p.W = ib.W; p.C = (int)po.cout_g; p.ctiles = p.C / 64;
    p.tiles_x = op.dwt_tiles_x; p.tiles_y = op.dwt_tiles_y; p.wbo = op.dwt_wbo; p.hb = op.dwt_hb; p.stages = op.dwt_stages;
    p.n_items = N * p.tiles_y * p.tiles_x * p.ctiles;
    const int grid = std::min(p.n_items, std::max(1, e->num_sms - e->reserve_sms));
    if (pair)                     launch_pdl(dwconv3_tma_kernel<2, 1>, grid, DWT_THREADS, op.dwt_smem, st, op.tmap_dw, p);
    else if (dw_dilation(po) == 2) launch_pdl(dwconv3_tma_kernel<1, 2>, grid, DWT_THREADS, op.dwt_smem, st, op.tmap_dw, p);
    else                          launch_pdl(dwconv3_tma_kernel<1, 1>, grid, DWT_THREADS, op.dwt_smem, st, op.tmap_dw, p);
}

int launch_conv(hp_engine* e, EngOp& op, int N, cudaStream_t st, bool u8_input)
{
    ConvPlan& pl = op.plan;
    ConvParams p = pl.prm;
    p.Nb = N;
    const int stem_R = op.launch == Launch::ConvStem && u8_input ? (int)op.po.R : 0;
    p.frames = e->cur_frames ? e->cur_frames : e->d_frames;
    if (op.launch == Launch::Halo) {
        HaloParams h = pl.hp;
        h.Nb = N;
        const int tiles = halo_shape(pl.halo_item, p.BN).tiles;
        const long items = ((long)N * h.tiles_x * h.tiles_y + tiles - 1) / tiles * h.groups * (h.cout_g_pad / p.BN);
        cudaLaunchAttribute at[1];
        const cudaLaunchConfig_t cfg = pdl_config((int)std::min<long>(e->num_sms - e->reserve_sms, items), CONV_THREADS, pl.smem, st, at);
        void* args[] = { (void*)&pl.tmap_x, (void*)&pl.tmap_b, (void*)&pl.tmap_o, (void*)&h };
        HP_CUDA_TRY(cudaLaunchKernelExC(&cfg, halo_kernel(p.BN, pl.halo_item, pl.halo_pool), args));
        return HP_OK;
    }
    p.m_tiles = (int)(((size_t)N * p.H * p.W + CONV_BLOCK_M - 1) / CONV_BLOCK_M);
    const int n_tiles = p.m_tiles * p.groups * (p.cout_g_pad / p.BN);
    const int grid = std::min(e->num_sms - e->reserve_sms, n_tiles);
    cudaLaunchAttribute at[1];
    const cudaLaunchConfig_t cfg = pdl_config(grid, CONV_THREADS, pl.smem, st, at);
    void* args[] = { (void*)&pl.tmap_a, (void*)&pl.tmap_b, (void*)&pl.tmap_o, (void*)&p };
    HP_CUDA_TRY(cudaLaunchKernelExC(&cfg, conv_kernel(e->dtype, p.res_mode != 0, p.BN, stem_R), args));
    return HP_OK;
}

bool collect_one(hp_engine* e, bool blocking)
{
    if (e->ev_tail >= e->ev_head) return false;
    const size_t n = e->ops.size();
    cudaEvent_t* set = e->ev.data() + (size_t)(e->ev_tail % hp_engine::EV_DEPTH) * (n + 1);
    if (!blocking && cudaEventQuery(set[n]) != cudaSuccess) { cudaGetLastError(); return false; }
    cudaEventSynchronize(set[n]);
    for (size_t i = 0; i < n; ++i) {
        float ms = 0.f;
        if (cudaEventElapsedTime(&ms, set[i], set[i + 1]) == cudaSuccess) e->op_ms_sum[i] += ms;
    }
    e->profiled_runs++;
    e->ev_tail++;
    return true;
}

void collect_profile(hp_engine* e)
{
    while (collect_one(e, true)) {}
}

template <typename T>
void launch_heads(hp_engine* e, const PackOp& po, int N, cudaStream_t st)
{
    if (e->heads_wait) cudaStreamWaitEvent(st, e->heads_wait, 0);
    const EngBuffer& a = e->bufs[po.in_buf];
    const EngBuffer& b = e->bufs[po.res_buf];
    const size_t t1 = (size_t)N * 17 * 5 * e->out_h * e->out_w, t2 = (size_t)N * 19 * 9 * e->out_h * e->out_w;
    pifpaf_head_kernel<T><<<(int)((t1 + 255) / 256), 256, 0, st>>>((const T*)a.d, a.channels, e->d_conf, N, a.H, a.W, 17, 5, e->out_h, e->out_w, 0);
    pifpaf_head_kernel<T><<<(int)((t2 + 255) / 256), 256, 0, st>>>((const T*)b.d, b.channels, e->d_paf, N, b.H, b.W, 19, 9, e->out_h, e->out_w, 1);
}

template <typename T>
void launch_ppn_head(hp_engine* e, const PackOp& po, int N, cudaStream_t st)
{
    const EngBuffer& a = e->bufs[po.in_buf];
    const int K = (int)po.cout_g, n_edge = (int)(po.groups * po.R * po.S);
    const size_t total = (size_t)N * (6 * K + n_edge) * e->out_h * e->out_w;
    ppn_head_kernel<T><<<(unsigned)((total + 255) / 256), 256, 0, st>>>((const T*)a.d, a.channels, e->d_conf, e->d_paf, N, e->out_h, e->out_w, K, n_edge,
                                                                        (float)((double)e->in_w / e->out_w), (float)((double)e->in_h / e->out_h),
                                                                        (float)e->in_w, (float)e->in_h);
}

template <typename T>
void launch_im2col_c4(hp_engine* e, const PackOp& po, int N, cudaStream_t st, bool u8_input)
{
    const EngBuffer& ob = e->bufs[po.out_buf];
    const int R = po.R ? (int)po.R : 3, stride = po.stride ? (int)po.stride : 1;
    const unsigned blocks = (unsigned)(((size_t)N * ob.H * ob.W * (ob.channels / 4) + 255) / 256);
    const void* in = u8_input ? (const void*)(e->cur_frames ? e->cur_frames : e->d_frames) : (const void*)e->d_input_f32;
    const float inv_s = std::is_same<T, int8_t>::value ? 1.0f / e->act_scale[po.out_buf] : 0.f;
    (u8_input ? im2col_c4_kernel<T, true> : im2col_c4_kernel<T, false>)<<<blocks, 256, 0, st>>>(
        in, (T*)ob.d, N, e->in_h, e->in_w, u8_input ? e->factor : 1.0, u8_input ? e->flip_rgb : 0, e->hdr.mean[0], e->hdr.mean[1], e->hdr.mean[2], R, stride,
        ob.H, ob.W, same_pad_before(e->in_h, R, stride), same_pad_before(e->in_w, R, stride), ob.channels, inv_s);
}

template <typename T>
void launch_dw_c4(hp_engine* e, const EngOp& op, int N, cudaStream_t st)
{
    const PackOp& po = op.po;
    const EngBuffer& ib = e->bufs[po.in_buf];
    const EngBuffer& ob = e->bufs[po.out_buf];
    const int C = (int)po.cout_g, K = (int)po.R, stride = po.stride ? (int)po.stride : 1, D = dw_dilation(po), span = (K - 1) * D + 1;
    const unsigned blocks = (unsigned)(((size_t)N * ob.H * ob.W * (C / 4) + 255) / 256);
    const bool i8 = std::is_same<T, int8_t>::value;
    const float* w = op.d_dw;
    dwconv_c4_kernel<T><<<blocks, 256, 0, st>>>((const T*)ib.d + po.in_ch_off, ib.channels, (T*)ob.d + po.out_ch_off, ob.channels, w, w + (size_t)K * K * C,
                                                w + (size_t)K * K * C + C, N, ib.H, ib.W, C, ob.H, ob.W, K, stride, D, same_pad_before(ib.H, span, stride),
                                                same_pad_before(ib.W, span, stride), i8 ? e->act_scale[po.in_buf] : 0.f, i8 ? 1.0f / e->act_scale[po.out_buf] : 0.f);
}

template <typename T>
void launch_maxpool_c4(hp_engine* e, const PackOp& po, int N, cudaStream_t st)
{
    const EngBuffer& ib = e->bufs[po.in_buf];
    const EngBuffer& ob = e->bufs[po.out_buf];
    const int C = (int)po.cout_g, K = po.R ? (int)po.R : 2;
    const unsigned blocks = (unsigned)(((size_t)N * ob.H * ob.W * (C / 4) + 255) / 256);
    maxpool_c4_kernel<T><<<blocks, 256, 0, st>>>((const T*)ib.d + po.in_ch_off, (T*)ob.d + po.out_ch_off, N, ib.H, ib.W, ib.channels, C, ob.channels, ob.H, ob.W,
                                                 K, same_pad_before(ib.H, K, 2), same_pad_before(ib.W, K, 2));
}

int run_graph(hp_engine* e, int N, bool u8_input, cudaStream_t st, int first = 0, int last = -1)
{
    if (last < 0) last = (int)e->ops.size() - 1;
    const bool prof = e->profiling && first == 0 && last == (int)e->ops.size() - 1;
    cudaEvent_t* evset = nullptr;
    if (prof) {
        while (collect_one(e, false)) {}
        if (e->ev_head - e->ev_tail >= hp_engine::EV_DEPTH) collect_one(e, true);
        evset = e->ev.data() + (size_t)(e->ev_head % hp_engine::EV_DEPTH) * (e->ops.size() + 1);
        cudaEventRecord(evset[0], st);
    }
    tl_use_pdl = e->use_pdl;
    const uint8_t* frames = e->cur_frames ? e->cur_frames : e->d_frames;
    for (int oi = first; oi <= last; ++oi) {
        EngOp& op = e->ops[oi];
        const PackOp& po = op.po;
        const int K = (int)po.R, stride = po.stride ? (int)po.stride : 1;
        switch (op.launch) {
        case Launch::None:
            break;
        case Launch::StemOrIm2col:
            if (u8_input) break;
            [[fallthrough]];
        case Launch::Im2col: {
            const EngBuffer& ob = e->bufs[po.out_buf];
            const int R = K ? K : 3, chunks = ob.channels / 64;
            const dim3 blocks((unsigned)(((size_t)N * ob.H * ob.W + 255) / 256), (unsigned)chunks);
            const int ph = same_pad_before(e->in_h, R, stride), pw = same_pad_before(e->in_w, R, stride);
#define HP_IM2COL(U8, RR, SRC, FAC, FLIP) im2col3_kernel<U8, RR><<<blocks, 256, 0, st>>>(SRC, ob.d, N, e->in_h, e->in_w, FAC, FLIP, \
                e->hdr.mean[0], e->hdr.mean[1], e->hdr.mean[2], stride, ob.H, ob.W, ph, pw, chunks)
            if (u8_input) { if (R == 3) HP_IM2COL(true, 3, frames, e->factor, e->flip_rgb); else HP_IM2COL(true, 7, frames, e->factor, e->flip_rgb); }
            else          { if (R == 3) HP_IM2COL(false, 3, e->d_input_f32, 1.0, 0); else HP_IM2COL(false, 7, e->d_input_f32, 1.0, 0); }
#undef HP_IM2COL
            break;
        }
        case Launch::Conv: case Launch::ConvStem: case Launch::Halo:
            launch_conv(e, op, N, st, u8_input);
            break;
        case Launch::DwTma:
            launch_dw_tma(e, op, nullptr, N, st);
            break;
        case Launch::DwTmaPair:
            launch_dw_tma(e, op, &e->ops[oi + 1], N, st);
            break;
        case Launch::DwCol: {
            const EngBuffer& ib = e->bufs[po.in_buf];
            const EngBuffer& ob = e->bufs[po.out_buf];
            const int C = (int)po.cout_g, D = dw_dilation(po), Hs = (ib.H + D - 1) / D;
            const size_t base = ((size_t)N * D * ib.W * (C / 4) + 255) / 256;
            int chunks = (int)((4 * (size_t)e->num_sms + base - 1) / base);
            chunks = std::max(1, std::min(chunks, std::max(1, Hs / 4)));
            const int rows = (Hs + chunks - 1) / chunks;
            chunks = (Hs + rows - 1) / rows;
            const size_t tot = (size_t)N * D * chunks * ib.W * (C / 4);
#define HP_DWCOL(DD) dwconv3_col_kernel<DD><<<(unsigned)((tot + 255) / 256), 256, 0, st>>>(ib.d + po.in_ch_off, ib.channels, ob.d + po.out_ch_off, \
                ob.channels, op.d_dw, op.d_dw + (size_t)9 * C, op.d_dw + (size_t)9 * C + C, N, ib.H, ib.W, C, rows, chunks)
            if (D == 2) HP_DWCOL(2); else HP_DWCOL(1);
#undef HP_DWCOL
            break;
        }
        case Launch::DwStrip: {
            const EngBuffer& ib = e->bufs[po.in_buf];
            const EngBuffer& ob = e->bufs[po.out_buf];
            const int C = (int)po.cout_g;
            const size_t total = (size_t)N * ob.H * ((ob.W + DW_STRIP - 1) / DW_STRIP) * (C / 8);
            const int blocks = (int)((total + 255) / 256);
            const float* dw = op.d_dw;
#define HP_DW(KK, SS) dwconv_kernel<KK, SS><<<blocks, 256, 0, st>>>(ib.d + po.in_ch_off, ib.channels, ob.d + po.out_ch_off, ob.channels, dw, \
                dw + (size_t)KK * KK * C, dw + (size_t)KK * KK * C + C, N, ib.H, ib.W, C, ob.H, ob.W, same_pad_before(ib.H, KK, SS), same_pad_before(ib.W, KK, SS))
            if (K == 3) HP_DW(3, 2);
            else if (stride == 2) HP_DW(1, 2);
            else HP_DW(1, 1);
#undef HP_DW
            break;
        }
        case Launch::MaxPool: {
            const EngBuffer& ib = e->bufs[po.in_buf];
            const EngBuffer& ob = e->bufs[po.out_buf];
            const int C = (int)po.cout_g;
            const int blocks = (int)(((size_t)N * ob.H * ob.W * (C / 8) + 255) / 256);
            if (K == 3)
                maxpool2_kernel<3><<<blocks, 256, 0, st>>>(ib.d + po.in_ch_off, ob.d + po.out_ch_off, N, ib.H, ib.W, ib.channels, C, ob.channels, ob.H, ob.W,
                                                           same_pad_before(ib.H, 3, 2), same_pad_before(ib.W, 3, 2));
            else
                maxpool2_kernel<2><<<blocks, 256, 0, st>>>(ib.d + po.in_ch_off, ob.d + po.out_ch_off, N, ib.H, ib.W, ib.channels, C, ob.channels, ob.H, ob.W,
                                                           same_pad_before(ib.H, 2, 2), same_pad_before(ib.W, 2, 2));
            break;
        }
        case Launch::Heads:
            if (e->dtype == HP_DTYPE_TF32) launch_heads<float>(e, po, N, st); else launch_heads<__half>(e, po, N, st);
            break;
        case Launch::PpnHead:
            if (e->dtype == HP_DTYPE_TF32) launch_ppn_head<float>(e, po, N, st); else launch_ppn_head<__half>(e, po, N, st);
            break;
        case Launch::Im2colC4:
            if (e->dtype == HP_DTYPE_INT8) launch_im2col_c4<int8_t>(e, po, N, st, u8_input); else launch_im2col_c4<float>(e, po, N, st, u8_input);
            break;
        case Launch::DwC4:
            if (e->dtype == HP_DTYPE_INT8) launch_dw_c4<int8_t>(e, op, N, st); else launch_dw_c4<float>(e, op, N, st);
            break;
        case Launch::MaxPoolC4:
            if (e->dtype == HP_DTYPE_INT8) launch_maxpool_c4<int8_t>(e, po, N, st); else launch_maxpool_c4<float>(e, po, N, st);
            break;
        }
        e->launches += kernels_launched(op.launch, u8_input);
        if (prof) cudaEventRecord(evset[oi + 1], st);
    }
    if (prof) e->ev_head++;
    if (e->override_conf && e->override_paf && last == (int)e->ops.size() - 1) {
        const size_t plane = (size_t)e->out_h * e->out_w;
        HP_CUDA_TRY(cudaMemcpyAsync(e->d_conf, e->override_conf, N * e->hdr.conf_channels * plane * sizeof(float), cudaMemcpyDeviceToDevice, st));
        HP_CUDA_TRY(cudaMemcpyAsync(e->d_paf, e->override_paf, N * e->hdr.paf_channels * plane * sizeof(float), cudaMemcpyDeviceToDevice, st));
    }
    HP_CUDA_TRY(cudaGetLastError());
    e->last_N = N;
    return HP_OK;
}

void free_engine(hp_engine* e)
{
    if (!e) return;
// ... 71 lines not shown
    if (device < 0 || device >= ndev || in_w <= 0 || in_h <= 0 || max_batch <= 0) { set_error("hp_engine_create: bad device/size/batch"); return HP_ERR_ARG; }
    if (pack_bytes < sizeof(PackHeader)) { set_error("hp_engine_create: pack too small"); return HP_ERR_ARG; }
    PackHeader hdr;
    memcpy(&hdr, pack, sizeof(hdr));
    if (memcmp(hdr.magic, PACK_MAGIC, 8) != 0 || hdr.version != PACK_VERSION) { set_error("hp_engine_create: not an HPB2PACK v%u model pack", PACK_VERSION); return HP_ERR_ARG; }
    if (hdr.n_buffers == 0 || hdr.n_buffers > 65536 || hdr.n_ops == 0 || hdr.n_ops > 65536 || hdr.blob_floats > ((uint64_t)1 << 34)) {
        set_error("hp_engine_create: implausible pack header (%u buffers, %u ops, %llu blob floats)", hdr.n_buffers, hdr.n_ops, (unsigned long long)hdr.blob_floats);
        return HP_ERR_ARG;
    }
    const uint32_t n_scales = hdr.reserved[0];
    if (n_scales != 0 && n_scales != hdr.n_buffers) { set_error("hp_engine_create: the pack's scale table has %u entries for %u buffers", n_scales, hdr.n_buffers); return HP_ERR_ARG; }
    const size_t need = sizeof(PackHeader) + (size_t)hdr.n_buffers * sizeof(PackBuffer) + (size_t)hdr.n_ops * sizeof(PackOp) + (size_t)hdr.blob_floats * sizeof(float) +
                        (size_t)n_scales * sizeof(float);
    if (pack_bytes < need) { set_error("hp_engine_create: truncated pack (%zu < %zu bytes)", pack_bytes, need); return HP_ERR_ARG; }
    std::vector<float> act_scale;
    if (dtype == HP_DTYPE_INT8) {
        if (hdr.head_type != 0) { set_error("hp_engine_create: the INT8 engine has no OpenPifPaf or PPN heads (pack head_type %u)", hdr.head_type); return HP_ERR_ARG; }
        if (n_scales == 0) { set_error("hp_engine_create: the pack has no INT8 scale table (export it with an INT8 calibration)"); return HP_ERR_ARG; }
        act_scale.resize(n_scales);
        memcpy(act_scale.data(), (const uint8_t*)pack + need - (size_t)n_scales * sizeof(float), (size_t)n_scales * sizeof(float));
        for (uint32_t b = 0; b < n_scales; ++b)
            if (!(std::isfinite(act_scale[b]) && act_scale[b] > 0.f)) { set_error("hp_engine_create: INT8 scale of buffer %u is %g (needs a finite value > 0)", b, (double)act_scale[b]); return HP_ERR_ARG; }
        const PackOp* vops = (const PackOp*)((const uint8_t*)pack + sizeof(PackHeader) + (size_t)hdr.n_buffers * sizeof(PackBuffer));
        for (uint32_t i = 0; i < hdr.n_ops; ++i) {
            PackOp po;
            memcpy(&po, vops + i, sizeof(po));
            if (po.type == OP_MAXPOOL2 && po.in_buf < n_scales && po.out_buf < n_scales && act_scale[po.in_buf] != act_scale[po.out_buf]) {
                set_error("hp_engine_create: INT8 max-pool op %u reads buffer %u (scale %g) but writes buffer %u (scale %g); they must be equal", i, po.in_buf,
                          (double)act_scale[po.in_buf], po.out_buf, (double)act_scale[po.out_buf]);
                return HP_ERR_ARG;
            }
        }
    }
    {
        const PackOp* vops = (const PackOp*)((const uint8_t*)pack + sizeof(PackHeader) + (size_t)hdr.n_buffers * sizeof(PackBuffer));
        auto in_blob = [&](uint64_t off, uint64_t count) { return off <= hdr.blob_floats && count <= hdr.blob_floats - off; };
        for (uint32_t i = 0; i < hdr.n_ops; ++i) {
            PackOp po;
            memcpy(&po, vops + i, sizeof(po));
            if (po.type == OP_DWCONV) {
                const uint32_t D = po.dilation ? po.dilation : 1;
                if (D > 2 || (D == 2 && (po.R != 3 || po.S != 3 || (po.stride ? po.stride : 1) != 1))) {
                    set_error("hp_engine_create: depthwise op %u has dilation %u with a %ux%u filter at stride %u (dilation 2 needs 3x3 at stride 1; "
                              "otherwise 0 or 1)", i, po.dilation, po.R, po.S, po.stride ? po.stride : 1);
                    return HP_ERR_ARG;
                }
            } else if (po.dilation != 0) {
                set_error("hp_engine_create: op %u (type %u) has dilation %u; only depthwise ops take one", i, po.type, po.dilation);
                return HP_ERR_ARG;
            }
            if (po.type != OP_CONV && po.type != OP_DWCONV) continue;
            const uint64_t lim = 1u << 16;
            const bool dw = po.type == OP_DWCONV;
            const uint64_t G = dw ? 1 : po.groups, co = po.cout_g, ci = dw ? 1 : po.cin_g, R = po.R, S = po.S;
            if (!dw && (G == 0 || co == 0 || ci == 0 || R % 2 == 0 || S % 2 == 0)) {
                set_error("hp_engine_create: conv op %u has a %ux%u filter, %u groups of %u -> %u channels (the conv kernels take odd "
                          "filter sizes and at least one group and channel)", i, po.R, po.S, po.groups, po.cin_g, po.cout_g);
                return HP_ERR_ARG;
            }
            if (G == 0 || co == 0 || ci == 0 || R == 0 || S == 0 || G > lim || co > lim || ci > lim || R > 15 || S > 15 ||
                !in_blob(po.w_off, G * co * ci * R * S) || !in_blob(po.b_off, G * co) || !in_blob(po.a_off, G * co)) {
                set_error("hp_engine_create: op %u names weights outside the pack (groups %u, cout %u, cin %u, %ux%u)", i, po.groups, po.cout_g, po.cin_g, po.R, po.S);
                return HP_ERR_ARG;
            }
        }
    }
    HP_CUDA_TRY(cudaSetDevice(device));
    cudaDeviceProp prop;
    HP_CUDA_TRY(cudaGetDeviceProperties(&prop, device));
    if (prop.major != 9) { set_error("hp_engine_create: device is sm_%d%d; this engine is wgmma/TMA code for sm_90a only", prop.major, prop.minor); return HP_ERR_UNSUPPORTED; }

    hp_engine* e = new hp_engine();
    e->device = device; e->dtype = dtype; e->in_h = in_h; e->in_w = in_w; e->max_batch = max_batch;
    e->factor = factor; e->flip_rgb = flip_rgb; e->hdr = hdr; e->num_sms = prop.multiProcessorCount;
    e->act_scale = std::move(act_scale);
    EngOptions& opt = e->opt;
    if (const char* v = getenv("HPB_HALO")) opt.halo = strcmp(v, "all") == 0 ? EngOptions::HALO_ALL : EngOptions::HALO_NONE;
    opt.halo_wide = !getenv("HPB_HALO_NARROW");
    opt.halo_tma_store = !getenv("HPB_HALO_REG_EPILOGUE");
    opt.conv_tma_store = !getenv("HPB_CONV_REG_EPILOGUE");
    opt.stem3 = !getenv("HPB_NO_STEM3");
    opt.pool_fuse = !getenv("HPB_NO_POOL_FUSE");
    opt.dw1_fuse = !getenv("HPB_NO_DW1_FUSE");
    opt.dw_pair = !getenv("HPB_NO_DW_DUAL");
    opt.dw_tma = !getenv("HPB_NO_DW_TMA");
    const char* rs = getenv("HPB_PIFPAF_RESERVE_SMS");
    opt.pifpaf_reserve_sms = std::max(0, std::min(rs ? atoi(rs) : std::min(max_batch, 16), e->num_sms / 2));
    const uint8_t* ptr = (const uint8_t*)pack + sizeof(PackHeader);
    const PackBuffer* pb = (const PackBuffer*)ptr;
    const PackOp* pops = (const PackOp*)(ptr + hdr.n_buffers * sizeof(PackBuffer));
    std::vector<float> blob(hdr.blob_floats);
    memcpy(blob.data(), (const uint8_t*)pops + hdr.n_ops * sizeof(PackOp), hdr.blob_floats * sizeof(float));

    int rc = HP_OK;
    auto fail = [&](int code) { free_engine(e); return code; };
    if (cudaStreamCreateWithFlags(&e->stream, cudaStreamNonBlocking) != cudaSuccess) { set_error("cudaStreamCreate failed"); return fail(HP_ERR_CUDA); }
    e->bufs.resize(hdr.n_buffers);
    for (uint32_t i = 0; i < hdr.n_buffers; ++i) {
        EngBuffer& b = e->bufs[i];
        b.channels = (int)pb[i].channels; b.down = (int)pb[i].down_shift;
        b.H = in_h; b.W = in_w;
        for (int d = 0; d < b.down; ++d) { b.H = (b.H + 1) / 2; b.W = (b.W + 1) / 2; }
        if (b.channels % 8) { set_error("engine: buffer %u has %d channels (need a multiple of 8)", i, b.channels); return fail(HP_ERR_ARG); }
        const size_t bytes = (size_t)max_batch * b.H * b.W * b.channels * (size_t)elem_bytes(dtype);
        if (cudaMalloc(&b.d, bytes) != cudaSuccess) { set_error("engine: cudaMalloc(%zu) failed", bytes); return fail(HP_ERR_CUDA); }
        cudaMemset(b.d, 0, bytes);
    }
    e->out_h = in_h; e->out_w = in_w;
    for (uint32_t d = 0; d < hdr.out_down_shift; ++d) { e->out_h = (e->out_h + 1) / 2; e->out_w = (e->out_w + 1) / 2; }
    if (hdr.head_type == 1) { e->out_h = 2 * e->out_h - 1; e->out_w = 2 * e->out_w - 1; }
    if (cudaMalloc(&e->d_conf, (size_t)max_batch * hdr.conf_channels * e->out_h * e->out_w * sizeof(float)) != cudaSuccess ||
        cudaMalloc(&e->d_paf, (size_t)max_batch * hdr.paf_channels * e->out_h * e->out_w * sizeof(float)) != cudaSuccess ||
        cudaMalloc(&e->d_frames, (size_t)max_batch * in_h * in_w * 3 + 16) != cudaSuccess ||
        cudaMallocHost(&e->pin_frames, (size_t)max_batch * in_h * in_w * 3) != cudaSuccess) {
        set_error("engine: output/frame allocation failed");
        return fail(HP_ERR_CUDA);
    }
    e->ops.resize(hdr.n_ops);
    size_t max_smem = 0;
    const bool f16 = dtype == HP_DTYPE_F16;
    for (uint32_t i = 0; i < hdr.n_ops; ++i) {
        EngOp& op = e->ops[i];
        op.po = pops[i];
        const PackOp& po = op.po;
        if ((po.type != OP_IM2COL3 && po.in_buf >= hdr.n_buffers) ||
            (po.out_mode != OUT_F32_NCHW_SPLIT && po.type != OP_PIFPAF_HEAD && po.type != OP_PPN_HEAD && po.out_buf >= hdr.n_buffers)) {
            set_error("engine: op %u references a missing buffer", i);
            return fail(HP_ERR_ARG);
        }
        if (po.type == OP_CONV) {
            rc = build_conv_plan(e, op, blob.data());
            if (rc) return fail(rc);
            max_smem = std::max(max_smem, op.plan.smem);
            e->flops_per_frame += op.plan.flops_per_frame;
        } else if (po.type == OP_IM2COL3) {
            const int stride = po.stride ? (int)po.stride : 1;
            const int R = po.R ? (int)po.R : 3;
            if (e->bufs[po.out_buf].channels != round_up(R * R * 3, 64) || e->bufs[po.out_buf].down != (stride == 2 ? 1 : 0) || stride > 2 || (R != 3 && R != 7)) {
                set_error("engine: im2col buffer must hold roundup(R*R*3,64) channels at the stem resolution");
                return fail(HP_ERR_ARG);
            }
            op.launch = f16 ? Launch::Im2col : Launch::Im2colC4;
        } else if (po.type == OP_DWCONV) {
            const int C = (int)po.cout_g, K = (int)po.R, stride = po.stride ? (int)po.stride : 1;
            const EngBuffer& ib = e->bufs[po.in_buf];
            const EngBuffer& ob = e->bufs[po.out_buf];
            if (C % 8 || (K != 1 && K != 3) || po.S != po.R || stride < 1 || stride > 2 || ob.down != ib.down + (stride == 2 ? 1 : 0) ||
                (int)po.in_ch_off + C > ib.channels || (int)po.out_ch_off + C > ob.channels || po.in_ch_off % 8 || po.out_ch_off % 8) {
                set_error("engine: bad depthwise op %u", i);
                return fail(HP_ERR_ARG);
            }
            std::vector<float> w((size_t)K * K * C + 2 * (size_t)C);
            for (int c = 0; c < C; ++c) {
                for (int t = 0; t < K * K; ++t) w[(size_t)t * C + c] = blob[po.w_off + (size_t)c * K * K + t];
                w[(size_t)K * K * C + c] = blob[po.b_off + c];
                w[(size_t)K * K * C + C + c] = blob[po.a_off + c];
            }
            if (cudaMalloc(&op.d_dw, w.size() * sizeof(float)) != cudaSuccess ||
                cudaMemcpy(op.d_dw, w.data(), w.size() * sizeof(float), cudaMemcpyHostToDevice) != cudaSuccess) {
                set_error("engine: depthwise weight upload failed");
                return fail(HP_ERR_CUDA);
            }
            e->flops_per_frame += 2.0 * ob.H * ob.W * C * K * K;
            op.launch = f16 ? (K == 3 && stride == 1 ? Launch::DwCol : Launch::DwStrip) : Launch::DwC4;
        } else if (po.type == OP_MAXPOOL2) {
            const EngBuffer& ib = e->bufs[po.in_buf];
// ... 8 lines not shown
            if (hdr.head_type != 1 || po.res_buf >= hdr.n_buffers || hdr.conf_channels != 85 || hdr.paf_channels != 171 ||
                e->bufs[po.in_buf].channels < 340 || e->bufs[po.res_buf].channels < 684 ||
                e->bufs[po.in_buf].down != (int)hdr.out_down_shift || e->bufs[po.res_buf].down != (int)hdr.out_down_shift) {
                set_error("engine: bad pifpaf head op %u", i);
                return fail(HP_ERR_ARG);
            }
            op.launch = Launch::Heads;
        } else if (po.type == OP_PPN_HEAD) {
            const uint64_t K = po.cout_g, n_edge = (uint64_t)po.groups * po.R * po.S;
            const EngBuffer& ib = e->bufs[po.in_buf];
            if (hdr.head_type != 2) { set_error("engine: PPN head op %u in a pack with head_type %u (needs 2)", i, hdr.head_type); return fail(HP_ERR_ARG); }
            if (ib.down != (int)hdr.out_down_shift) {
                set_error("engine: PPN head op %u reads buffer %u at down-shift %d but the outputs are at %u", i, po.in_buf, ib.down, hdr.out_down_shift);
                return fail(HP_ERR_ARG);
            }
            if (K < 18 || K > 4096 || n_edge == 0 || n_edge > (1u << 20)) {
                set_error("engine: PPN head op %u has K=%llu key points and %llu edge channels (needs K >= 18 for the COCO limb table)", i,
                          (unsigned long long)K, (unsigned long long)n_edge);
                return fail(HP_ERR_ARG);
            }
            if ((uint64_t)ib.channels < 6 * K + n_edge) {
                set_error("engine: PPN head op %u reads %llu channels of a %d-channel buffer", i, (unsigned long long)(6 * K + n_edge), ib.channels);
                return fail(HP_ERR_ARG);
            }
            if (hdr.conf_channels != 6 * K || hdr.paf_channels != n_edge) {
                set_error("engine: PPN head op %u writes %llu box and %llu edge channels but the pack header says conf %u / paf %u", i,
                          (unsigned long long)(6 * K), (unsigned long long)n_edge, hdr.conf_channels, hdr.paf_channels);
                return fail(HP_ERR_ARG);
            }
            op.launch = Launch::PpnHead;
            e->ppn_K = (int)K; e->ppn_E = (int)po.groups; e->ppn_nh = (int)po.R; e->ppn_nw = (int)po.S;
        } else {
            set_error("engine: unknown op type %u", po.type);
            return fail(HP_ERR_UNSUPPORTED);
        }
    }
    for (EngOp& c : e->ops) {
        const PackOp& po = c.po;
        const int R = (int)po.R;
        if (dtype != HP_DTYPE_F16 || c.launch != Launch::Conv || !po.im2col_input || po.res_mode || po.out_mode != OUT_F16_NHWC || po.S != po.R || !(R == 7 || (R == 3 && opt.stem3))) continue;
        for (EngOp& m : e->ops) {
            if (m.po.type != OP_IM2COL3 || m.po.out_buf != po.in_buf) continue;
            if ((int)(m.po.R ? m.po.R : 3) != R || po.cin_g != 3) break;
            ConvParams& p = c.plan.prm;
            const int stride = m.po.stride ? (int)m.po.stride : 1;
            p.in_h = in_h; p.in_w = in_w; p.stem_stride = stride;
            p.stem_pad_h = same_pad_before(in_h, R, stride); p.stem_pad_w = same_pad_before(in_w, R, stride);
            p.factor = factor; p.flip = flip_rgb;
            p.mean[0] = hdr.mean[0]; p.mean[1] = hdr.mean[1]; p.mean[2] = hdr.mean[2];
            c.launch = Launch::ConvStem;
            m.launch = Launch::StemOrIm2col;
            break;
        }
    }
    for (size_t i = 0; opt.pool_fuse && i + 1 < e->ops.size(); ++i) {
        EngOp& c = e->ops[i]; EngOp& m = e->ops[i + 1];
        if (c.launch != Launch::Halo || c.plan.halo_pool || !c.plan.monotone_act || m.po.type != OP_MAXPOOL2 || (m.po.R != 0 && m.po.R != 2)) continue;
        const EngBuffer& cb = e->bufs[c.po.out_buf];
        const EngBuffer& pb = e->bufs[m.po.out_buf];
        const int C = (int)c.po.groups * (int)c.po.cout_g;
        if (m.po.in_buf != c.po.out_buf || m.po.in_ch_off != c.po.out_ch_off || (int)m.po.cout_g != C || c.plan.hp.cout_g_pad != c.plan.hp.cout_g ||
            (cb.H & 1) || (cb.W & 1) || pb.H != cb.H / 2 || pb.W != cb.W / 2 || (int)m.po.out_ch_off + C > pb.channels) continue;
        bool other_reader = false;
        for (size_t k = 0; k < e->ops.size(); ++k)
            if (k != i + 1 && reads_buffer(e->ops[k].po, c.po.out_buf)) other_reader = true;
        if (other_reader) continue;
        c.plan.hp.out = pb.d; c.plan.hp.out_ld = pb.channels; c.plan.hp.out_ch_off = (int)m.po.out_ch_off;
        if (int rc = set_halo_item(e, c, pick_halo_item(e, c, true), true)) return fail(rc);
        max_smem = std::max(max_smem, c.plan.smem);
        m.launch = Launch::None;
        e->bufs[c.po.out_buf].fused_away = true;
    }
    for (size_t i = 0; opt.dw1_fuse && i + 1 < e->ops.size(); ++i) {
        EngOp& c = e->ops[i]; EngOp& d = e->ops[i + 1];
        if ((c.launch != Launch::Conv && c.launch != Launch::ConvStem) || d.launch != Launch::DwStrip || d.po.R != 1 || (d.po.stride ? d.po.stride : 1) != 1) continue;
        const ConvParams& cp = c.plan.prm;
        const int Ctot = (int)c.po.groups * (int)c.po.cout_g;
        if (c.po.out_mode != OUT_F16_NHWC || cp.cout_g_pad != cp.cout_g || cp.cout_g % 16 ||
            d.po.in_buf != c.po.out_buf || d.po.in_ch_off != c.po.out_ch_off || (int)d.po.cout_g != Ctot || d.po.out_buf == c.po.out_buf) continue;
        if (d.po.out_buf == c.po.in_buf) {
            if (cp.R != 1 || cp.S != 1 || cp.cin_g != cp.cout_g || cp.BN != cp.cout_g || (int)d.po.out_ch_off != cp.in_ch_off) continue;
        }
        if (c.po.res_mode && d.po.out_buf == c.po.res_buf) continue;
        bool safe = true, rewritten = false;
        for (size_t k = i + 2; k < e->ops.size() && safe && !rewritten; ++k) {
            const PackOp& q = e->ops[k].po;
            if (reads_buffer(q, c.po.out_buf)) safe = false;
            else if (q.type != OP_IM2COL3 && q.type != OP_PIFPAF_HEAD && q.type != OP_PPN_HEAD && q.out_mode != OUT_F32_NCHW_SPLIT && q.out_buf == c.po.out_buf) {
                const int qc = q.type == OP_CONV ? (int)q.groups * (int)q.cout_g : (int)q.cout_g;
                if (q.out_ch_off <= c.po.out_ch_off && (int)q.out_ch_off + qc >= (int)c.po.out_ch_off + Ctot) rewritten = true; else safe = false;
            }
        }
        if (!safe) continue;
        const EngBuffer& ob = e->bufs[d.po.out_buf];
        if ((int)d.po.out_ch_off + Ctot > ob.channels) continue;
        c.plan.prm.out = ob.d; c.plan.prm.out_ld = ob.channels; c.plan.prm.out_ch_off = (int)d.po.out_ch_off;
        c.plan.prm.post_w = d.d_dw; c.plan.prm.post_b = d.d_dw + Ctot; c.plan.prm.post_a = d.d_dw + 2 * (size_t)Ctot;
        d.launch = Launch::None;
        if (!rewritten) e->bufs[c.po.out_buf].fused_away = true;
    }
    for (EngOp& c : e->ops) {
        if (c.launch != Launch::Conv && c.launch != Launch::ConvStem) continue;
        if (int rc = set_conv_tma_store(e, c)) return fail(rc);
        max_smem = std::max(max_smem, c.plan.smem);
    }
    size_t dwt_max = 0;
    for (EngOp& a : e->ops) {
        const PackOp& po = a.po;
        if (!opt.dw_tma || a.launch != Launch::DwCol || po.cout_g % 64 || po.in_buf == po.out_buf) continue;
        const EngBuffer& ib = e->bufs[po.in_buf];
        const int C = (int)po.cout_g, halo = 2 * dw_dilation(po);
        const int nx = (ib.W + 63 - halo) / (64 - halo), wbo = (ib.W + nx - 1) / nx, bw = wbo + halo;
        int hb = 2;
        for (int cand : { 8, 6, 4, 3, 2 }) {
            if (cand > std::max(2, ib.H) || (size_t)(cand + halo) * bw * 128 > (size_t)DWT_STAGE_MAX) continue;
            const size_t items = (size_t)e->max_batch * ((ib.H + cand - 1) / cand) * nx * (C / 64);
            hb = cand;
            if (items >= 2 * (size_t)e->num_sms) break;
        }
        const size_t stage = (size_t)(hb + halo) * bw * 128;
        if (stage > (size_t)DWT_STAGE_MAX) continue;
        a.dwt_stages = (int)std::min<size_t>(4, (200 * 1024) / stage);
        if (a.dwt_stages < 2) continue;
        a.dwt_wbo = wbo; a.dwt_hb = hb; a.dwt_tiles_x = nx; a.dwt_tiles_y = (ib.H + hb - 1) / hb;
        a.dwt_smem = a.dwt_stages * stage + 128 + 64;
        if (make_tmap_act_box(&a.tmap_dw, ib.d + po.in_ch_off, e->max_batch, ib.H, ib.W, C, ib.channels, bw, hb + halo, CU_TENSOR_MAP_SWIZZLE_NONE) != HP_OK) return fail(HP_ERR_CUDA);
        a.launch = Launch::DwTma;
        dwt_max = std::max(dwt_max, a.dwt_smem);
    }
    if (dwt_max > 0 && (cudaFuncSetAttribute(dwconv3_tma_kernel<1, 1>, cudaFuncAttributeMaxDynamicSharedMemorySize, (int)dwt_max) != cudaSuccess ||
                        cudaFuncSetAttribute(dwconv3_tma_kernel<2, 1>, cudaFuncAttributeMaxDynamicSharedMemorySize, (int)dwt_max) != cudaSuccess ||
                        cudaFuncSetAttribute(dwconv3_tma_kernel<1, 2>, cudaFuncAttributeMaxDynamicSharedMemorySize, (int)dwt_max) != cudaSuccess)) {
        set_error("engine: cannot opt in to %zu bytes of dynamic shared memory (depthwise)", dwt_max);
        return fail(HP_ERR_CUDA);
    }
    for (size_t i = 0; opt.dw_pair && i + 1 < e->ops.size(); ++i) {
        EngOp& a = e->ops[i]; EngOp& b = e->ops[i + 1];
        if (a.launch != Launch::DwTma || b.launch != Launch::DwTma || a.po.in_buf != b.po.in_buf || a.po.in_ch_off != b.po.in_ch_off ||
            a.po.cout_g != b.po.cout_g || a.po.out_buf != b.po.out_buf || dw_dilation(a.po) != 1 || dw_dilation(b.po) != 1) continue;
        a.launch = Launch::DwTmaPair;
        b.launch = Launch::None;
    }
    int launches = 0;
    for (const EngOp& o : e->ops) {
        if ((o.po.type == OP_CONV || o.po.type == OP_DWCONV || o.po.type == OP_MAXPOOL2) && o.launch != Launch::None) ++launches;
        e->step_kernels += kernels_launched(o.launch, true);
    }
    const double per_launch = launches ? e->flops_per_frame * e->max_batch / launches : 0.0;
    e->use_pdl = dtype == HP_DTYPE_F16 && launches > 0 && per_launch < 10e9;
    for (const EngOp& o : e->ops) {
        if (o.po.type != OP_CONV) continue;
        if (o.launch == Launch::Halo &&
            cudaFuncSetAttribute(halo_kernel(o.plan.prm.BN, o.plan.halo_item, o.plan.halo_pool), cudaFuncAttributeMaxDynamicSharedMemorySize, (int)max_smem) != cudaSuccess) {
            set_error("engine: cannot opt in to %zu bytes of dynamic shared memory (halo)", max_smem);
            return fail(HP_ERR_CUDA);
        }
        const int stem_R = o.launch == Launch::ConvStem ? (int)o.po.R : 0;
        for (int v = 0; v < 3; ++v)
            if ((v < 2 || stem_R) &&
                cudaFuncSetAttribute(conv_kernel(dtype, v == 1, o.plan.prm.BN, v == 2 ? stem_R : 0), cudaFuncAttributeMaxDynamicSharedMemorySize, (int)max_smem) != cudaSuccess) {
                set_error("engine: cannot opt in to %zu bytes of dynamic shared memory", max_smem);
                return fail(HP_ERR_CUDA);
            }
    }
    if (cudaDeviceSynchronize() != cudaSuccess) { set_error("hp_engine_create: device error during set-up: %s", cudaGetErrorString(cudaGetLastError())); return fail(HP_ERR_CUDA); }
    *out = e;
    return HP_OK;
}

void hp_engine_destroy(hp_engine* e) { free_engine(e); }

int hp_engine_info(const hp_engine* e, int* in_w, int* in_h, int* max_batch, int* c_conf, int* c_paf, int* out_h, int* out_w, double* flops_per_frame)
{
    if (!e) return HP_ERR_ARG;
    if (in_w) *in_w = e->in_w;
    if (in_h) *in_h = e->in_h;
    if (max_batch) *max_batch = e->max_batch;
    if (c_conf) *c_conf = (int)e->hdr.conf_channels;
    if (c_paf) *c_paf = (int)e->hdr.paf_channels;
    if (out_h) *out_h = e->out_h;
    if (out_w) *out_w = e->out_w;
    if (flops_per_frame) *flops_per_frame = e->flops_per_frame;
    return HP_OK;
}

int hp_engine_head_type(const hp_engine* e) { return e ? (int)e->hdr.head_type : HP_ERR_ARG; }

int hp_engine_infer_u8_host(hp_engine* e, const uint8_t* frames, int N)
{
    if (!e || !frames) { set_error("hp_engine_infer_u8_host: null argument"); return HP_ERR_ARG; }
    if (N <= 0 || N > e->max_batch) { set_error("Input batch size overflow: Yours@%d Max@%d", N, e->max_batch); return HP_ERR_BATCH; }
    HP_CUDA_TRY(cudaSetDevice(e->device));
    const size_t bytes = (size_t)N * e->in_h * e->in_w * 3;
    cudaPointerAttributes attr;
    const bool pinned = (cudaPointerGetAttributes(&attr, frames) == cudaSuccess && attr.type == cudaMemoryTypeHost);
    if (!pinned) cudaGetLastError();
    if (pinned) {
        HP_CUDA_TRY(cudaMemcpyAsync(e->d_frames, frames, bytes, cudaMemcpyHostToDevice, e->stream));
    } else {
        HP_CUDA_TRY(cudaStreamSynchronize(e->stream));
        memcpy(e->pin_frames, frames, bytes);
        HP_CUDA_TRY(cudaMemcpyAsync(e->d_frames, e->pin_frames, bytes, cudaMemcpyHostToDevice, e->stream));
    }
    return run_graph(e, N, true, e->stream);
}

int hp_engine_infer_u8_device(hp_engine* e, const uint8_t* d_frames, int N, void* stream)
{
    if (!e || !d_frames) { set_error("hp_engine_infer_u8_device: null argument"); return HP_ERR_ARG; }
    if (N <= 0 || N > e->max_batch) { set_error("Input batch size overflow: Yours@%d Max@%d", N, e->max_batch); return HP_ERR_BATCH; }
    HP_CUDA_TRY(cudaSetDevice(e->device));
    cudaStream_t st = stream ? (cudaStream_t)stream : e->stream;
    HP_CUDA_TRY(cudaMemcpyAsync(e->d_frames, d_frames, (size_t)N * e->in_h * e->in_w * 3, cudaMemcpyDeviceToDevice, st));
    return run_graph(e, N, true, st);
}

int hp_engine_infer_f32_host(hp_engine* e, const float* nchw, int N)
{
    if (!e || !nchw) { set_error("hp_engine_infer_f32_host: null argument"); return HP_ERR_ARG; }
    if (N <= 0 || N > e->max_batch) { set_error("Input batch size overflow: Yours@%d Max@%d", N, e->max_batch); return HP_ERR_BATCH; }
    HP_CUDA_TRY(cudaSetDevice(e->device));
    const size_t n = (size_t)e->max_batch * 3 * e->in_h * e->in_w;
    if (!e->d_input_f32) HP_CUDA_TRY(cudaMalloc(&e->d_input_f32, n * sizeof(float)));
    HP_CUDA_TRY(cudaMemcpyAsync(e->d_input_f32, nchw, (size_t)N * 3 * e->in_h * e->in_w * sizeof(float), cudaMemcpyHostToDevice, e->stream));
    return run_graph(e, N, false, e->stream);
}

static int frame_desc(const hp_engine* e, const uint8_t* src, int src_h, int src_w, int keep_ratio, FrameDesc& d)
{
    d = FrameDesc{ src, src_h, src_w, e->in_h, e->in_w, RZ_COPY, 0 };
    if (src_h == e->in_h && src_w == e->in_w) return HP_OK;
    if (keep_ratio) {
        const double h1 = e->in_w * (src_h / (double)src_w);
        const double w2 = e->in_h * (src_w / (double)src_h);
        if (h1 <= e->in_h) { d.rw = e->in_w; d.rh = (int)h1; } else { d.rw = (int)w2; d.rh = e->in_h; }
        if (d.rh <= 0 || d.rw <= 0) { set_error("degenerate letterbox: %dx%d into %dx%d", src_h, src_w, e->in_h, e->in_w); return HP_ERR_ARG; }
// ... 232 lines not shown
    auto done = [&](int rc) { cudaFree(d_amax); return rc; };
    if (cudaMemcpy(d_amax, absmax, (size_t)n_buffers * sizeof(float), cudaMemcpyHostToDevice) != cudaSuccess) { set_error("hp_engine_calibrate_u8: upload failed"); return done(HP_ERR_CUDA); }
    const size_t frame_bytes = (size_t)e->in_h * e->in_w * 3;
    for (int f0 = 0; f0 < N; f0 += e->max_batch) {
        const int n = std::min(e->max_batch, N - f0);
        memcpy(e->pin_frames, frames + (size_t)f0 * frame_bytes, (size_t)n * frame_bytes);
        if (cudaMemcpyAsync(e->d_frames, e->pin_frames, (size_t)n * frame_bytes, cudaMemcpyHostToDevice, e->stream) != cudaSuccess) { set_error("hp_engine_calibrate_u8: H2D failed"); return done(HP_ERR_CUDA); }
        for (int oi = 0; oi < (int)e->ops.size(); ++oi) {
            const int rc = run_graph(e, n, true, e->stream, oi, oi);
            if (rc) return done(rc);
            const PackOp& po = e->ops[oi].po;
            if (po.type == OP_PIFPAF_HEAD || po.type == OP_PPN_HEAD || (po.type == OP_CONV && po.out_mode == OUT_F32_NCHW_SPLIT)) continue;
            const EngBuffer& b = e->bufs[po.out_buf];
            const size_t cnt = (size_t)n * b.H * b.W * b.channels;
            absmax_f32_kernel<<<(unsigned)std::min<size_t>(1024, (cnt + 255) / 256), 256, 0, e->stream>>>((const float*)b.d, cnt, d_amax + po.out_buf);
        }
        if (cudaStreamSynchronize(e->stream) != cudaSuccess) { set_error("hp_engine_calibrate_u8: %s", cudaGetErrorString(cudaGetLastError())); return done(HP_ERR_CUDA); }
    }
    if (cudaMemcpy(absmax, d_amax, (size_t)n_buffers * sizeof(float), cudaMemcpyDeviceToHost) != cudaSuccess) { set_error("hp_engine_calibrate_u8: read-back failed"); return done(HP_ERR_CUDA); }
    return done(HP_OK);
}

int hp_pack_int8_calibrated(const void* pack, size_t pack_bytes)
{
    if (!pack || pack_bytes < sizeof(PackHeader)) return 0;
    PackHeader hdr;
    memcpy(&hdr, pack, sizeof(hdr));
    if (memcmp(hdr.magic, PACK_MAGIC, 8) != 0 || hdr.version != PACK_VERSION || hdr.n_buffers == 0 || hdr.reserved[0] != hdr.n_buffers ||
        hdr.n_buffers > 65536 || hdr.n_ops > 65536 || hdr.blob_floats > ((uint64_t)1 << 34))
        return 0;
    const size_t need = sizeof(PackHeader) + (size_t)hdr.n_buffers * sizeof(PackBuffer) + (size_t)hdr.n_ops * sizeof(PackOp) +
                        ((size_t)hdr.blob_floats + hdr.n_buffers) * sizeof(float);
    return pack_bytes >= need ? 1 : 0;
}

int hp_engine_debug_op_kernel(const hp_engine* e, int op, char* name, int cap)
{
    if (!e || op < 0 || op >= (int)e->ops.size() || !name || cap <= 0) { set_error("hp_engine_debug_op_kernel: bad argument"); return HP_ERR_ARG; }
    const EngOp& o = e->ops[op];
    const PackOp& po = o.po;
    const int BN = o.plan.prm.BN;
    const char* dt = e->dtype == HP_DTYPE_TF32 ? "tf32," : e->dtype == HP_DTYPE_INT8 ? "i8," : "f16,";
    const std::string c4 = e->dtype == HP_DTYPE_INT8 ? "_i8" : "_f32";
    std::string s;
    switch (o.launch) {
    case Launch::None: case Launch::StemOrIm2col: s = "none"; break;
    case Launch::Im2col: s = "im2col"; break;
    case Launch::Conv:
        s = std::string("conv<") + dt + std::to_string(BN) + (o.plan.prm.res_mode ? ",res>" : ">");
        break;
    case Launch::ConvStem: s = "conv<f16," + std::to_string(BN) + ",stem" + std::to_string(po.R) + ">"; break;
    case Launch::Halo:
        s = "halo<" + std::to_string(BN) + (o.plan.halo_pool ? ",pool" : "") +
            (o.plan.halo_item == HaloItem::Wide ? ",wide" : o.plan.halo_item == HaloItem::PingPong ? ",pp" : "") + ">";
        break;
    case Launch::DwTma: s = "dw_tma<1>"; break;
    case Launch::DwTmaPair: s = "dw_tma<2>"; break;
    case Launch::DwCol: s = "dw_col"; break;
    case Launch::DwStrip: s = "dw_strip<" + std::to_string(po.R) + "," + std::to_string(po.stride ? po.stride : 1) + ">"; break;
    case Launch::MaxPool: s = "maxpool<" + std::to_string(po.R ? po.R : 2) + ">"; break;
    case Launch::Heads: s = "heads"; break;
    case Launch::PpnHead: s = "ppn_head"; break;
    case Launch::Im2colC4: s = e->dtype == HP_DTYPE_INT8 ? "im2col_i8" : "im2col"; break;
    case Launch::DwC4: s = "dw" + c4; break;
    case Launch::MaxPoolC4: s = "maxpool" + c4; break;
    }
    if (po.type == OP_DWCONV && o.launch != Launch::None && dw_dilation(po) != 1) {
        const std::string d = "d" + std::to_string(dw_dilation(po));
        s = s.back() == '>' ? s.substr(0, s.size() - 1) + "," + d + ">" : s + "<" + d + ">";
    }
    if ((int)s.size() >= cap) { set_error("hp_engine_debug_op_kernel: %zu-character name, capacity %d", s.size(), cap); return HP_ERR_CAPACITY; }
    memcpy(name, s.c_str(), s.size() + 1);
    return HP_OK;
}

int hp_engine_debug_op_epilogue(const hp_engine* e, int op, int* tma_store)
{
    if (!e || op < 0 || op >= (int)e->ops.size() || !tma_store) { set_error("hp_engine_debug_op_epilogue: bad argument"); return HP_ERR_ARG; }
    const EngOp& o = e->ops[op];
    *tma_store = o.launch == Launch::Halo && o.plan.hp.tma_store ? 1 : 0;
    return HP_OK;
}

int hp_engine_debug_op_conv_epilogue(const hp_engine* e, int op, int* tma_store)
{
    if (!e || op < 0 || op >= (int)e->ops.size() || !tma_store) { set_error("hp_engine_debug_op_conv_epilogue: bad argument"); return HP_ERR_ARG; }
    const EngOp& o = e->ops[op];
    *tma_store = (o.launch == Launch::Conv || o.launch == Launch::ConvStem) && o.plan.prm.tma_store ? 1 : 0;
    return HP_OK;
}

int hp_engine_debug_uses_pdl(const hp_engine* e, int* pdl)
{
    if (!e || !pdl) { set_error("hp_engine_debug_uses_pdl: bad argument"); return HP_ERR_ARG; }
    *pdl = e->use_pdl ? 1 : 0;
    return HP_OK;
}

long long hp_engine_launch_count(const hp_engine* e) { return e ? e->launches : 0; }

int hp_engine_set_output_override(hp_engine* e, const float* d_conf, const float* d_paf)
{
    if (!e) return HP_ERR_ARG;
    e->override_conf = d_conf;
    e->override_paf = d_paf;
    return HP_OK;
}

int hp_engine_set_profiling(hp_engine* e, int enable)
{
    if (!e) return HP_ERR_ARG;
    HP_CUDA_TRY(cudaSetDevice(e->device));
    if (enable && e->ev.empty()) {
        e->ev.resize((e->ops.size() + 1) * hp_engine::EV_DEPTH);
        for (auto& ev : e->ev) HP_CUDA_TRY(cudaEventCreate(&ev));
    }
    if (enable) {
        e->op_ms_sum.assign(e->ops.size(), 0.0);
        e->profiled_runs = 0;
        e->ev_head = e->ev_tail = 0;
    } else {
        collect_profile(e);
    }
    e->profiling = enable != 0;
    return HP_OK;
}

int hp_engine_get_profile(hp_engine* e, double* ms_per_op, int* op_type, double* flops_per_op, int cap, int* n_ops, long long* runs)
{
    if (!e) return HP_ERR_ARG;
    HP_CUDA_TRY(cudaSetDevice(e->device));
    collect_profile(e);
    const int n = (int)e->ops.size();
    if (n_ops) *n_ops = n;
    if (runs) *runs = e->profiled_runs;
    if (cap < n) { set_error("hp_engine_get_profile: cap %d < %d ops", cap, n); return HP_ERR_CAPACITY; }
    for (int i = 0; i < n; ++i) {
        if (ms_per_op) ms_per_op[i] = (e->profiled_runs && i < (int)e->op_ms_sum.size()) ? e->op_ms_sum[i] / e->profiled_runs : 0.0;
        if (op_type) op_type[i] = (int)e->ops[i].po.type;
        if (flops_per_op) flops_per_op[i] = e->ops[i].po.type == OP_CONV ? e->ops[i].plan.flops_per_frame : 0.0;
    }
    return HP_OK;
}

int hp_paf_prepare(hp_paf* p, int N, int c_conf, int c_paf, int H, int W);
int hp_paf_state(const hp_paf* p, float* thresholds2, int* ints6);
int hp_paf_copy_results_host_async(hp_paf* p, hp_human* pin_humans, int* pin_counts_flags, int N, void* stream);
int hp_paf_grow_capacity(hp_paf* p, int flags);
int hp_pifpaf_process_device(hp_pifpaf* p, const float* d_pif, const float* d_paf, int N, int h, int w, void* stream);
int hp_pifpaf_pipeline_info(hp_pifpaf* p, void** stream, void** inputs_free_event, int* hcap);
int hp_pifpaf_copy_results_host_async(hp_pifpaf* p, hp_human* pin_humans, int* pin_counts_flags, int N, void* stream);
int hp_pifpaf_grow_capacity(hp_pifpaf* p, int flags);

#ifdef HPB_HALO_PHASES
int hp_debug_halo_phases(unsigned long long* out, int n, int reset)
{
    if (!out || n != HALO_PH_COUNT) { set_error("hp_debug_halo_phases: expected %d counters", (int)HALO_PH_COUNT); return HP_ERR_ARG; }
    HP_CUDA_TRY(cudaDeviceSynchronize());
    HP_CUDA_TRY(cudaMemcpyFromSymbol(out, g_halo_phases, sizeof(unsigned long long) * HALO_PH_COUNT));
    if (reset) {
        const unsigned long long zero[HALO_PH_COUNT] = {};
        HP_CUDA_TRY(cudaMemcpyToSymbol(g_halo_phases, zero, sizeof(zero)));
    }
    return HP_OK;
}
#endif
// ... 789 lines not shown
```

include/hyperpose_b200.h:

```cpp
#ifndef HYPERPOSE_B200_H
#define HYPERPOSE_B200_H

#include <stddef.h>
#include <stdint.h>

#ifdef __cplusplus
extern "C" {
#endif

#define HP_N_PARTS 18
#define HP_N_PAIRS 19

typedef enum hp_status {
    HP_OK = 0,
    HP_ERR_ARG = -1,
    HP_ERR_CAPACITY = -2,
    HP_ERR_UNSUPPORTED = -3,
    HP_ERR_CUDA = -4,
    HP_ERR_BATCH = -5
} hp_status;

typedef struct hp_body_part {
    int32_t has_value;
    float x, y, score;
// ... 25 lines not shown
int hp_paf_set_paf_thresh(hp_paf* p, float thresh);
int hp_paf_set_capacity(hp_paf* p, int max_peaks_per_part, int max_candidates_per_limb, int max_humans);

int hp_paf_process_host(hp_paf* p, const float* conf, const float* paf, int c_conf, int c_paf, int H, int W,
                        hp_human* out, int cap, int* n_out);
int hp_paf_process_host_batched(hp_paf* p, const float* conf, const float* paf, int N, int c_conf, int c_paf, int H, int W,
                                hp_human* out, int cap, int* n_out);
int hp_paf_process_device(hp_paf* p, const float* d_conf, const float* d_paf, int N, int c_conf, int c_paf, int H, int W,
                          void* stream);
int hp_paf_fetch(hp_paf* p, hp_human* out, int cap, int* n_out, int N);

int hp_paf_debug_peaks(hp_paf* p, int frame, hp_peak* out, int cap, int* n_out);
int hp_paf_debug_connections(hp_paf* p, int frame, int pair_id, hp_connection* out, int cap, int* n_out);
long long hp_paf_launch_count(const hp_paf* p);
int hp_paf_debug_timing(hp_paf* p, unsigned long long* out, int N);
#define HP_PAF_PLAN_FIELDS 8
int hp_paf_debug_plan(hp_paf* p, int* out, int n);
int hp_paf_copy_results_device(hp_paf* p, hp_human* d_humans, int* d_counts, int N, int cap, void* stream);

typedef struct hp_pifpaf hp_pifpaf;
int hp_pifpaf_create(hp_pifpaf** out, int net_h, int net_w, float thresh, int device);
void hp_pifpaf_destroy(hp_pifpaf* p);
int hp_pifpaf_process_host(hp_pifpaf* p, const float* pif, const float* paf, int N, int h, int w, hp_human* out, int cap, int* n_out);
int hp_pifpaf_process_device(hp_pifpaf* p, const float* d_pif, const float* d_paf, int N, int h, int w, void* stream);
int hp_pifpaf_fetch(hp_pifpaf* p, hp_human* out, int cap, int* n_out, int N);
long long hp_pifpaf_launch_count(const hp_pifpaf* p);
int hp_pifpaf_debug_counts(hp_pifpaf* p, int frame, int* out7);
int hp_pifpaf_debug_hr(hp_pifpaf* p, int frame, int field, float* out);

typedef struct hp_ppn hp_ppn;
int hp_ppn_create(hp_ppn** out, int net_w, int net_h, float point_thresh, float limb_thresh, float nms_thresh, int device);
void hp_ppn_destroy(hp_ppn* p);
int hp_ppn_set_point_thresh(hp_ppn* p, float thresh);
int hp_ppn_set_limb_thresh(hp_ppn* p, float thresh);
int hp_ppn_set_nms_thresh(hp_ppn* p, float thresh);
int hp_ppn_process_host(hp_ppn* p, const float* conf_point, const float* x, const float* y, const float* w, const float* h,
                        const float* edge, int N, int K, int gh, int gw, int E, int nh, int nw, hp_human* out, int cap, int* n_out);
int hp_ppn_process_device(hp_ppn* p, const float* d_conf_point, const float* d_x, const float* d_y, const float* d_w, const float* d_h,
                          const float* d_edge, int N, int K, int gh, int gw, int E, int nh, int nw, void* stream);
int hp_ppn_process_device_strided(hp_ppn* p, const float* d_conf_point, const float* d_x, const float* d_y, const float* d_w, const float* d_h,
                                  const float* d_edge, int N, int K, int gh, int gw, int E, int nh, int nw, size_t box_frame_stride,
                                  size_t edge_frame_stride, void* stream);
int hp_ppn_fetch(hp_ppn* p, hp_human* out, int cap, int* n_out, int N);
long long hp_ppn_launch_count(const hp_ppn* p);

typedef struct hp_engine hp_engine;

int hp_engine_create(hp_engine** out, const void* pack, size_t pack_bytes, int in_w, int in_h, int max_batch,
                     double factor, int flip_rgb, int device);
#define HP_DTYPE_F16 0
#define HP_DTYPE_TF32 1
#define HP_DTYPE_INT8 2
int hp_engine_create_ex(hp_engine** out, const void* pack, size_t pack_bytes, int in_w, int in_h, int max_batch,
                        double factor, int flip_rgb, int device, int dtype);
int hp_engine_dtype(const hp_engine* e);
int hp_pack_int8_calibrated(const void* pack, size_t pack_bytes);
int hp_engine_calibrate_u8(hp_engine* e, const uint8_t* frames, int N, float* absmax, int n_buffers);
void hp_engine_destroy(hp_engine* e);
int hp_engine_info(const hp_engine* e, int* in_w, int* in_h, int* max_batch, int* c_conf, int* c_paf, int* out_h, int* out_w,
                   double* flops_per_frame);
int hp_engine_infer_u8_host(hp_engine* e, const uint8_t* frames, int N);
int hp_engine_infer_u8_device(hp_engine* e, const uint8_t* d_frames, int N, void* stream);
int hp_engine_stage_frame_u8(hp_engine* e, int slot, const uint8_t* frame, int src_h, int src_w, int keep_ratio);
int hp_engine_infer_staged(hp_engine* e, int N);
int hp_engine_debug_read_frames(hp_engine* e, uint8_t* out, int N);
int hp_engine_infer_f32_host(hp_engine* e, const float* nchw, int N);
int hp_engine_outputs(hp_engine* e, const float** d_conf, const float** d_paf, void** stream);
int hp_engine_read_outputs_host(hp_engine* e, float* conf, float* paf, int N);
int hp_engine_read_outputs_frames(hp_engine* e, float* const* conf_frames, float* const* paf_frames, int N, int publish);
int hp_engine_head_type(const hp_engine* e);
int hp_handoff_enable(int on);
int hp_handoff_stats(long long* published, long long* hits, long long* batch_parses, long long* misses);
int hp_engine_copy_outputs_device(hp_engine* e, float* d_conf, float* d_paf, int N, void* stream);
int hp_engine_sync(hp_engine* e);
long long hp_engine_launch_count(const hp_engine* e);
int hp_engine_debug_read_buffer(hp_engine* e, int buf, void* out_f16, int N, int* H, int* W, int* C);
int hp_engine_debug_write_buffer(hp_engine* e, int buf, const void* in_f16, int N);
int hp_engine_debug_run_ops(hp_engine* e, int first_op, int last_op, int N);
int hp_engine_debug_read_buffer_raw(hp_engine* e, int buf, void* out, int N);
int hp_engine_debug_write_outputs(hp_engine* e, const float* conf, const float* paf, int N);
int hp_engine_debug_op_kernel(const hp_engine* e, int op, char* name, int cap);
int hp_engine_debug_op_epilogue(const hp_engine* e, int op, int* tma_store);
int hp_engine_debug_op_conv_epilogue(const hp_engine* e, int op, int* tma_store);
int hp_engine_debug_uses_pdl(const hp_engine* e, int* pdl);

int hp_engine_set_output_override(hp_engine* e, const float* d_conf, const float* d_paf);
int hp_engine_set_profiling(hp_engine* e, int enable);
int hp_engine_get_profile(hp_engine* e, double* ms_per_op, int* op_type, double* flops_per_op, int cap, int* n_ops, long long* runs);

int hp_pose_run_u8_host(hp_engine* e, hp_paf* parser, const uint8_t* frames, int N, hp_human* out, int cap, int* n_out);
int hp_pose_submit_u8_host(hp_engine* e, hp_paf* parser, const uint8_t* frames, int N, int* ticket);
int hp_pose_submit_u8_device(hp_engine* e, hp_paf* parser, const uint8_t* d_frames, int N, int* ticket);
int hp_pose_collect(hp_engine* e, int ticket, hp_human* out, int cap, int* n_out);
int hp_pose_stats(const hp_engine* e, long long* graph_captures, long long* graph_launches);
int hp_pose_submit_pifpaf_u8_host(hp_engine* e, hp_pifpaf* decoder, const uint8_t* frames, int N, int* ticket);
int hp_pose_submit_pifpaf_u8_device(hp_engine* e, hp_pifpaf* decoder, const uint8_t* d_frames, int N, int* ticket);
typedef struct hp_frame_u8 { const uint8_t* data; int32_t height, width; } hp_frame_u8;
int hp_pose_submit_frames_u8_host(hp_engine* e, hp_paf* parser, const hp_frame_u8* frames, int N, int keep_ratio, int* ticket);
int hp_pose_submit_frames_u8_device(hp_engine* e, hp_paf* parser, const hp_frame_u8* frames, int N, int keep_ratio, int* ticket);
int hp_pose_submit_pifpaf_frames_u8_host(hp_engine* e, hp_pifpaf* decoder, const hp_frame_u8* frames, int N, int keep_ratio, int* ticket);
int hp_pose_submit_pifpaf_frames_u8_device(hp_engine* e, hp_pifpaf* decoder, const hp_frame_u8* frames, int N, int keep_ratio, int* ticket);
int hp_pose_submit_ppn_u8_host(hp_engine* e, hp_ppn* parser, const uint8_t* frames, int N, int* ticket);
int hp_pose_submit_ppn_u8_device(hp_engine* e, hp_ppn* parser, const uint8_t* d_frames, int N, int* ticket);
int hp_pose_submit_ppn_frames_u8_host(hp_engine* e, hp_ppn* parser, const hp_frame_u8* frames, int N, int keep_ratio, int* ticket);
int hp_pose_submit_ppn_frames_u8_device(hp_engine* e, hp_ppn* parser, const hp_frame_u8* frames, int N, int keep_ratio, int* ticket);
typedef struct hp_frame_yuv420 {
    const uint8_t *y, *u, *v;
    int32_t height, width;
    int32_t pitch_y, pitch_uv;
    int32_t uv_step;
} hp_frame_yuv420;
int hp_pose_submit_frames_yuv420_host(hp_engine* e, hp_paf* parser, const hp_frame_yuv420* frames, int N, int keep_ratio, int* ticket);
int hp_pose_submit_frames_yuv420_device(hp_engine* e, hp_paf* parser, const hp_frame_yuv420* frames, int N, int keep_ratio, int* ticket);
int hp_pose_submit_pifpaf_frames_yuv420_host(hp_engine* e, hp_pifpaf* decoder, const hp_frame_yuv420* frames, int N, int keep_ratio, int* ticket);
int hp_pose_submit_pifpaf_frames_yuv420_device(hp_engine* e, hp_pifpaf* decoder, const hp_frame_yuv420* frames, int N, int keep_ratio, int* ticket);
int hp_pose_submit_ppn_frames_yuv420_host(hp_engine* e, hp_ppn* parser, const hp_frame_yuv420* frames, int N, int keep_ratio, int* ticket);
int hp_pose_submit_ppn_frames_yuv420_device(hp_engine* e, hp_ppn* parser, const hp_frame_yuv420* frames, int N, int keep_ratio, int* ticket);
typedef enum hp_pixel_format {
    HP_PIX_BGR = 0, HP_PIX_RGB, HP_PIX_BGRA, HP_PIX_RGBA, HP_PIX_GRAY,
    HP_PIX_YUYV, HP_PIX_UYVY, HP_PIX_YVYU
} hp_pixel_format;
typedef struct hp_frame_interleaved {
    const uint8_t* data;
    int32_t height, width;
    int32_t pitch;
    int32_t format;
} hp_frame_interleaved;
int hp_pose_submit_frames_interleaved_host(hp_engine* e, hp_paf* parser, const hp_frame_interleaved* frames, int N, int keep_ratio, int* ticket);
int hp_pose_submit_frames_interleaved_device(hp_engine* e, hp_paf* parser, const hp_frame_interleaved* frames, int N, int keep_ratio, int* ticket);
int hp_pose_submit_pifpaf_frames_interleaved_host(hp_engine* e, hp_pifpaf* decoder, const hp_frame_interleaved* frames, int N, int keep_ratio, int* ticket);
int hp_pose_submit_pifpaf_frames_interleaved_device(hp_engine* e, hp_pifpaf* decoder, const hp_frame_interleaved* frames, int N, int keep_ratio, int* ticket);
int hp_pose_submit_ppn_frames_interleaved_host(hp_engine* e, hp_ppn* parser, const hp_frame_interleaved* frames, int N, int keep_ratio, int* ticket);
int hp_pose_submit_ppn_frames_interleaved_device(hp_engine* e, hp_ppn* parser, const hp_frame_interleaved* frames, int N, int keep_ratio, int* ticket);
int hp_pose_submit_frames_yuv420_rotated_host(hp_engine* e, hp_paf* parser, const hp_frame_yuv420* frames, const int32_t* rotation, int N,
                                              int keep_ratio, int* ticket);
int hp_pose_submit_frames_yuv420_rotated_device(hp_engine* e, hp_paf* parser, const hp_frame_yuv420* frames, const int32_t* rotation, int N,
                                                int keep_ratio, int* ticket);
int hp_pose_submit_pifpaf_frames_yuv420_rotated_host(hp_engine* e, hp_pifpaf* decoder, const hp_frame_yuv420* frames, const int32_t* rotation,
                                                     int N, int keep_ratio, int* ticket);
int hp_pose_submit_pifpaf_frames_yuv420_rotated_device(hp_engine* e, hp_pifpaf* decoder, const hp_frame_yuv420* frames, const int32_t* rotation,
                                                       int N, int keep_ratio, int* ticket);
int hp_pose_submit_ppn_frames_yuv420_rotated_host(hp_engine* e, hp_ppn* parser, const hp_frame_yuv420* frames, const int32_t* rotation, int N,
                                                  int keep_ratio, int* ticket);
int hp_pose_submit_ppn_frames_yuv420_rotated_device(hp_engine* e, hp_ppn* parser, const hp_frame_yuv420* frames, const int32_t* rotation, int N,
                                                    int keep_ratio, int* ticket);
int hp_pose_submit_frames_interleaved_rotated_host(hp_engine* e, hp_paf* parser, const hp_frame_interleaved* frames, const int32_t* rotation,
                                                   int N, int keep_ratio, int* ticket);
int hp_pose_submit_frames_interleaved_rotated_device(hp_engine* e, hp_paf* parser, const hp_frame_interleaved* frames, const int32_t* rotation,
                                                     int N, int keep_ratio, int* ticket);
int hp_pose_submit_pifpaf_frames_interleaved_rotated_host(hp_engine* e, hp_pifpaf* decoder, const hp_frame_interleaved* frames,
                                                          const int32_t* rotation, int N, int keep_ratio, int* ticket);
int hp_pose_submit_pifpaf_frames_interleaved_rotated_device(hp_engine* e, hp_pifpaf* decoder, const hp_frame_interleaved* frames,
                                                            const int32_t* rotation, int N, int keep_ratio, int* ticket);
int hp_pose_submit_ppn_frames_interleaved_rotated_host(hp_engine* e, hp_ppn* parser, const hp_frame_interleaved* frames,
                                                       const int32_t* rotation, int N, int keep_ratio, int* ticket);
int hp_pose_submit_ppn_frames_interleaved_rotated_device(hp_engine* e, hp_ppn* parser, const hp_frame_interleaved* frames,
                                                         const int32_t* rotation, int N, int keep_ratio, int* ticket);
int hp_pose_debug_read_slot_frames(hp_engine* e, int ticket, uint8_t* out, int N);
int hp_pifpaf_pipeline_info(hp_pifpaf* p, void** stream, void** inputs_free_event, int* hcap);
int hp_pifpaf_copy_results_host_async(hp_pifpaf* p, hp_human* pin_humans, int* pin_counts_flags, int N, void* stream);
int hp_pifpaf_grow_capacity(hp_pifpaf* p, int flags);
int hp_paf_prepare(hp_paf* p, int N, int c_conf, int c_paf, int H, int W);
int hp_paf_state(const hp_paf* p, float* thresholds2, int* ints6);
int hp_paf_copy_results_host_async(hp_paf* p, hp_human* pin_humans, int* pin_counts_flags, int N, void* stream);
int hp_paf_grow_capacity(hp_paf* p, int flags);
int hp_ppn_prepare(hp_ppn* p, int N, int K, int gh, int gw, int E, int nh, int nw);
// ... 21 lines not shown
```

Before: 1131.

## Chain two trailing 1x1 convs into the wide halo conv epilogue

Adds a chained form of the wide halo conv kernel. After the 3x3 conv's accumulators are activated, they are staged in shared memory and two following 1x1 convs (a grouped 128->128 and a final head conv) run as in-kernel wgmma GEMMs, with the result written directly to the head output. This removes two kernel launches and the round trips of the intermediate activations through global memory in the OpenPose head stages. In exchange the kernel holds the input box slot longer and does serial extra GEMMs per tile, which may lower pipelining and occupancy. The fusion applies only when strict shape and dead-buffer checks pass, and can be disabled with an environment variable.

```diff
diff --git a/hyperpose_b200/capi.py b/hyperpose_b200/capi.py
--- a/hyperpose_b200/capi.py
+++ b/hyperpose_b200/capi.py
@@ -189,7 +189,7 @@
     "hp_paf_grow_capacity", "hp_pool_create", "hp_pool_destroy", "hp_pool_size", "hp_pool_set_capacity", "hp_pool_run_u8_host",
     "hp_pool_set_output_override", "hp_pool_launch_count", "hp_default_device", "hp_handoff_device_of",
     "hp_engine_create_ex", "hp_engine_dtype", "hp_pose_submit_u8_device", "hp_engine_debug_op_kernel",
-    "hp_engine_debug_op_epilogue", "hp_engine_debug_op_conv_epilogue", "hp_engine_debug_uses_pdl",
+    "hp_engine_debug_op_epilogue", "hp_engine_debug_op_conv_epilogue", "hp_engine_debug_op_chained", "hp_engine_debug_uses_pdl",
     "hp_engine_debug_read_buffer_raw", "hp_engine_debug_write_outputs",
     "hp_engine_calibrate_u8", "hp_pack_int8_calibrated",
     "hp_pose_submit_frames_u8_host", "hp_pose_submit_frames_u8_device", "hp_pose_submit_pifpaf_frames_u8_host",
@@ -275,6 +275,7 @@
     L.hp_engine_debug_op_kernel.argtypes = [vp, C.c_int, C.c_char_p, C.c_int]
     L.hp_engine_debug_op_epilogue.argtypes = [vp, C.c_int, ip]
     L.hp_engine_debug_op_conv_epilogue.argtypes = [vp, C.c_int, ip]
+    L.hp_engine_debug_op_chained.argtypes = [vp, C.c_int, ip]
     L.hp_engine_debug_uses_pdl.argtypes = [vp, ip]
     L.hp_engine_debug_read_buffer_raw.argtypes = [vp, C.c_int, vp, C.c_int]
     L.hp_engine_debug_write_outputs.argtypes = [vp, vp, vp, C.c_int]
@@ -483,6 +484,11 @@
         check(lib().hp_engine_debug_op_conv_epilogue(self._h, op, C.byref(v)))
         return "tma" if v.value else "reg"
 
+    def debug_op_chained(self, op: int) -> bool:
+        v = C.c_int(0)
+        check(lib().hp_engine_debug_op_chained(self._h, op, C.byref(v)))
+        return bool(v.value)
+
     def debug_uses_pdl(self) -> bool:
         v = C.c_int(0)
         check(lib().hp_engine_debug_uses_pdl(self._h, C.byref(v)))
diff --git a/hyperpose_b200/csrc/conv_wgmma.cuh b/hyperpose_b200/csrc/conv_wgmma.cuh
--- a/hyperpose_b200/csrc/conv_wgmma.cuh
+++ b/hyperpose_b200/csrc/conv_wgmma.cuh
@@ -785,6 +785,12 @@
     __half* out; int out_ld, out_ch_off;
     int tma_store;
     int stage_bytes;
+    const float* c1_bias; const float* c1_alpha;
+    const float* c2_bias; const float* c2_alpha;
+    int c2_split, c2_cout;
+    int c2_mode;
+    void* c2_out; void* c2_out2;
+    int c2_out_ld, c2_out_ch_off, c2_plane_split;
 };
 
 enum class HaloItem { Narrow, Wide, PingPong };
@@ -884,6 +890,37 @@
     }
 }
 
+template <int BN>
+__device__ __forceinline__ void halo_stage_block(const float (&acc)[BN / 2], const float* bias, const float* alpha, uint32_t slot, int warp, int lane)
+{
+    constexpr int kSliceBytes = 64 * 128;
+    const int col0 = 2 * (lane & 3);
+    const int r = lane & 7, i = lane >> 3;
+#pragma unroll
+    for (int jb = 0; jb < BN / 32; ++jb) {
+        float2 b[4], a[4];
+#pragma unroll
+        for (int k = 0; k < 4; ++k) {
+            const int c = 8 * (4 * jb + k) + col0;
+            b[k] = __ldg((const float2*)(bias + c));
+            a[k] = __ldg((const float2*)(alpha + c));
+        }
+#pragma unroll
+        for (int h = 0; h < 2; ++h) {
+            uint32_t v[4];
+#pragma unroll
+            for (int k = 0; k < 4; ++k) {
+                float a0 = acc[4 * (4 * jb + k) + 2 * h] + b[k].x, a1 = acc[4 * (4 * jb + k) + 2 * h + 1] + b[k].y;
+                a0 = a0 > 0.f ? a0 : a0 * a[k].x;
+                a1 = a1 > 0.f ? a1 : a1 * a[k].y;
+                v[k] = ptx::half2_bits(__floats2half2_rn(a0, a1));
+            }
+            const int j = 4 * jb + i, row = (warp & 3) * 16 + 8 * h + r;
+            ptx::stmatrix_x4(slot + (uint32_t)((j >> 3) * kSliceBytes + row * 128 + (((j & 7) ^ r) << 4)), v[0], v[1], v[2], v[3]);
+        }
+    }
+}
+
 template <int BN, bool kPool, int kBlocks, int kSlots, bool kWait>
 __device__ __forceinline__ void halo_epilogue_tma(const float (&acc)[kBlocks][BN / 2], const HaloParams& p, const CUtensorMap* tmap_o, uint32_t stage,
                                                   int n, int y0, int x0, int g, int n0, int row_base, int warp, int lane, bool leader HALO_PH_PARAM)
@@ -924,30 +961,7 @@
                                    ptx::half2_bits(__floats2half2_rn(a0, a1)));
             }
         } else {
-            const int r = lane & 7, i = lane >> 3;
-#pragma unroll
-            for (int jb = 0; jb < BN / 32; ++jb) {
-                float2 b[4], a[4];
-#pragma unroll
-                for (int k = 0; k < 4; ++k) {
-                    const int c = 8 * (4 * jb + k) + col0;
-                    b[k] = __ldg((const float2*)(bias + c));
-                    a[k] = __ldg((const float2*)(alpha + c));
-                }
-#pragma unroll
-                for (int h = 0; h < 2; ++h) {
-                    uint32_t v[4];
-#pragma unroll
-                    for (int k = 0; k < 4; ++k) {
-                        float a0 = acc[m][4 * (4 * jb + k) + 2 * h] + b[k].x, a1 = acc[m][4 * (4 * jb + k) + 2 * h + 1] + b[k].y;
-                        a0 = a0 > 0.f ? a0 : a0 * a[k].x;
-                        a1 = a1 > 0.f ? a1 : a1 * a[k].y;
-                        v[k] = ptx::half2_bits(__floats2half2_rn(a0, a1));
-                    }
-                    const int j = 4 * jb + i, row = (warp & 3) * 16 + 8 * h + r;
-                    ptx::stmatrix_x4(slot + (uint32_t)((j >> 3) * kSliceBytes + row * 128 + (((j & 7) ^ r) << 4)), v[0], v[1], v[2], v[3]);
-                }
-            }
+            halo_stage_block<BN>(acc[m], bias, alpha, slot, warp, lane);
         }
         ptx::fence_proxy_async();
         ptx::named_barrier_sync(bar_id, 128);
@@ -1005,12 +1019,108 @@
     halo_epilogue<BN, kPool, kShape.blocks>(acc, p, n, y0, x0, g, n0, row_base, warp, lane);
 }
 
-template <int BN, bool kPool, HaloItem kItem>
+template <int N>
+__device__ __forceinline__ void halo_chain_gemm(float (&acc)[2][64], uint32_t stage, const uint8_t* s_b, uint64_t* b_full, uint64_t* b_empty,
+                                                RingPos& b, int num_stages, int lane)
+{
+    float (&d0)[N / 2] = *reinterpret_cast<float (*)[N / 2]>(&acc[0][0]);
+    float (&d1)[N / 2] = *reinterpret_cast<float (*)[N / 2]>(&acc[1][0]);
+    int used[2];
+#pragma unroll
+    for (int kc = 0; kc < 2; ++kc) {
+        const uint64_t db = ptx::make_sw128_kmajor_desc(ptx::smem_u32(s_b + (size_t)b.slot * 128 * 128));
+        const uint64_t da0 = ptx::make_sw128_kmajor_desc(stage + (uint32_t)(kc * 64 * 128));
+        const uint64_t da1 = ptx::make_sw128_kmajor_desc(stage + (uint32_t)(128 * 128 + kc * 64 * 128));
+        ptx::mbar_wait(ptx::smem_u32(b_full + b.slot), b.phase);
+        ptx::fence_acc(d0);
+        ptx::fence_acc(d1);
+        ptx::wgmma_fence();
+#pragma unroll
+        for (int k = 0; k < 4; ++k) {
+            ptx::wgmma<__half, N>(d0, da0 + (uint64_t)(k * 2), db + (uint64_t)(k * 2), (kc | k) != 0 ? 1u : 0u);
+            ptx::wgmma<__half, N>(d1, da1 + (uint64_t)(k * 2), db + (uint64_t)(k * 2), (kc | k) != 0 ? 1u : 0u);
+        }
+        ptx::wgmma_commit();
+        ptx::fence_acc(d0);
+        ptx::fence_acc(d1);
+        used[kc] = b.slot;
+        b.step(num_stages);
+    }
+    ptx::wgmma_wait<0>();
+    ptx::fence_acc(d0);
+    ptx::fence_acc(d1);
+    if (lane == 0) {
+        ptx::mbar_arrive(ptx::smem_u32(b_empty + used[0]));
+        ptx::mbar_arrive(ptx::smem_u32(b_empty + used[1]));
+    }
+}
+
+__device__ __forceinline__ void halo_chain(float (&acc)[2][64], const HaloParams& p, uint32_t stage, const uint8_t* s_b, uint64_t* b_full,
+                                           uint64_t* b_empty, RingPos& b, bool store, int n, int y0, int x0, int g, int nt, int warp, int lane)
+{
+    const int bar_id = warp >> 2;
+    ptx::named_barrier_sync(bar_id, 128);
+    halo_stage_block<128>(acc[0], p.bias + g * p.cout_g_pad, p.alpha + g * p.cout_g_pad, stage, warp, lane);
+    halo_stage_block<128>(acc[1], p.bias + g * p.cout_g_pad, p.alpha + g * p.cout_g_pad, stage + 128 * 128, warp, lane);
+    ptx::fence_proxy_async();
+    ptx::named_barrier_sync(bar_id, 128);
+    halo_chain_gemm<128>(acc, stage, s_b, b_full, b_empty, b, p.num_stages, lane);
+    ptx::named_barrier_sync(bar_id, 128);
+    halo_stage_block<128>(acc[0], p.c1_bias + nt * 128, p.c1_alpha + nt * 128, stage, warp, lane);
+    halo_stage_block<128>(acc[1], p.c1_bias + nt * 128, p.c1_alpha + nt * 128, stage + 128 * 128, warp, lane);
+    ptx::fence_proxy_async();
+    ptx::named_barrier_sync(bar_id, 128);
+    halo_chain_gemm<64>(acc, stage, s_b, b_full, b_empty, b, p.num_stages, lane);
+    if (!store) return;
+    const int lo = nt ? p.c2_split : 0, hi = nt ? p.c2_cout : p.c2_split;
+    const int col0 = 2 * (lane & 3), ox = x0 + (lane >> 2);
+    const bool pair_ok = ((p.c2_out_ch_off | p.c2_out_ld) & 1) == 0;
+#pragma unroll
+    for (int m = 0; m < 2; ++m) {
+#pragma unroll
+        for (int h = 0; h < 2; ++h) {
+            const int oy = y0 + 8 * m + 2 * (warp & 3) + h;
+            if (oy >= p.H || ox >= p.W) continue;
+            const size_t pix = ((size_t)n * p.H + oy) * p.W + ox;
+#pragma unroll
+            for (int j = 0; j < 8; ++j) {
+                const int c = 8 * j + col0;
+                const bool e0 = c >= lo && c < hi, e1 = c + 1 >= lo && c + 1 < hi;
+                if (!e0 && !e1) continue;
+                float a0 = acc[m][4 * j + 2 * h] + __ldg(p.c2_bias + c), a1 = acc[m][4 * j + 2 * h + 1] + __ldg(p.c2_bias + c + 1);
+                a0 = a0 > 0.f ? a0 : a0 * __ldg(p.c2_alpha + c);
+                a1 = a1 > 0.f ? a1 : a1 * __ldg(p.c2_alpha + c + 1);
+                if (p.c2_mode == OUT_F16_NHWC) {
+                    const __half2 h2 = __floats2half2_rn(a0, a1);
+                    __half* o = (__half*)p.c2_out + pix * p.c2_out_ld + p.c2_out_ch_off + c;
+                    if (e0 && e1 && pair_ok) *(__half2*)o = h2;
+                    else { if (e0) o[0] = __low2half(h2); if (e1) o[1] = __high2half(h2); }
+                } else {
+#pragma unroll
+                    for (int e = 0; e < 2; ++e) {
+                        if (!(e ? e1 : e0)) continue;
+                        const int ch = c + e;
+                        const float y = e ? a1 : a0;
+                        if (ch < p.c2_plane_split) {
+                            ((float*)p.c2_out)[(((size_t)n * p.c2_plane_split + ch) * p.H + oy) * p.W + ox] = y;
+                        } else {
+                            const int c2 = ch - p.c2_plane_split, n2 = p.c2_cout - p.c2_plane_split;
+                            ((float*)p.c2_out2)[(((size_t)n * n2 + c2) * p.H + oy) * p.W + ox] = y;
+                        }
+                    }
+                }
+            }
+        }
+    }
+}
+
+template <int BN, bool kPool, HaloItem kItem, bool kChain = false>
 __global__ void __launch_bounds__(CONV_THREADS, 1)
 conv_halo_kernel(const __grid_constant__ CUtensorMap tmap_x, const __grid_constant__ CUtensorMap tmap_b, const __grid_constant__ CUtensorMap tmap_o,
-                 const HaloParams p)
+                 const HaloParams p, const __grid_constant__ CUtensorMap tmap_c1, const __grid_constant__ CUtensorMap tmap_c2)
 {
     static_assert(!(kItem == HaloItem::Wide && kPool), "the pooled epilogue pairs pixel rows of one m64 block; it has no wide form");
+    static_assert(!kChain || (kItem == HaloItem::Wide && BN == 128), "the chained epilogue is a form of the wide item at BN = 128");
     static_assert(kItem != HaloItem::PingPong || BN == 64 || BN == 128, "the ping-pong item is built for the VGG trunk's widths, BN = 64 and 128");
     constexpr HaloShape kShape = halo_shape(kItem, BN);
     constexpr int B_BYTES = BN * 128;
@@ -1039,7 +1149,11 @@
     if (threadIdx.x == 0) {
         ptx::prefetch_tmap(&tmap_x);
         ptx::prefetch_tmap(&tmap_b);
-        if (kTmaForm && p.tma_store) ptx::prefetch_tmap(&tmap_o);
+        if (kTmaForm && p.tma_store && !kChain) ptx::prefetch_tmap(&tmap_o);
+        if (kChain) {
+            ptx::prefetch_tmap(&tmap_c1);
+            ptx::prefetch_tmap(&tmap_c2);
+        }
         for (int i = 0; i < kShape.box_slots; ++i) {
             ptx::mbar_init(ptx::smem_u32(a_full + i), 1);
             ptx::mbar_init(ptx::smem_u32(a_empty + i), kShape.slot_warps);
@@ -1100,6 +1214,17 @@
                         const uint32_t fb = ptx::smem_u32(b_full + b.slot);
                         ptx::mbar_expect_tx(fb, (uint32_t)B_BYTES);
                         ptx::tma_load_2d(ptx::smem_u32(s_b + (size_t)b.slot * B_BYTES), &tmap_b, fb, tap * p.cin_g + c * CONV_BLOCK_K, g * p.cout_g_pad + n0);
+                        b.step(p.num_stages);
+                    }
+                }
+                if constexpr (kChain) {
+                    const int nt = g * n_tiles_g + n0 / BN;
+                    for (int k = 0; k < 4; ++k) {
+                        ptx::mbar_wait(ptx::smem_u32(b_empty + b.slot), b.phase ^ 1);
+                        const uint32_t fb = ptx::smem_u32(b_full + b.slot), dst = ptx::smem_u32(s_b + (size_t)b.slot * B_BYTES);
+                        ptx::mbar_expect_tx(fb, (uint32_t)(k < 2 ? 128 * 128 : 64 * 128));
+                        if (k < 2) ptx::tma_load_2d(dst, &tmap_c1, fb, k * CONV_BLOCK_K, nt * 128);
+                        else ptx::tma_load_2d(dst, &tmap_c2, fb, nt * 128 + (k - 2) * CONV_BLOCK_K, 0);
                         b.step(p.num_stages);
                     }
                 }
@@ -1192,7 +1317,8 @@
                 for (int m = 0; m < kShape.blocks; ++m) ptx::fence_acc(acc[m]);
                 if (lane == 0) {
                     ptx::mbar_arrive(ptx::smem_u32(b_empty + prev));
-                    if (kItem == HaloItem::Wide && tma && leader && c == chunks - 1) held = a.slot;
+                    if (kChain && c == chunks - 1) {}
+                    else if (kItem == HaloItem::Wide && tma && leader && c == chunks - 1) held = a.slot;
                     else ptx::mbar_arrive(ptx::smem_u32(a_empty + a.slot));
                 }
                 a.step(kShape.box_slots);
@@ -1201,6 +1327,14 @@
             HALO_PH_MARK(t_epi);
             int n, y0, x0;
             tile_pos(sp + box, n, y0, x0);
+            if constexpr (kChain) {
+                const int last = (a.slot + kShape.box_slots - 1) % kShape.box_slots;
+                halo_chain(acc, p, ptx::smem_u32(s_box + (size_t)(last * kShape.tiles + box) * p.box_bytes), s_b, b_full, b_empty, b, n < p.Nb,
+                           n, y0, x0, g, g * n_tiles_g + n0 / BN, warp, lane);
+                if (lane == 0) ptx::mbar_arrive(ptx::smem_u32(a_empty + last));
+                HALO_PH_ADD(HALO_PH_EPILOGUE, t_epi);
+                continue;
+            }
             if (kItem == HaloItem::Wide && n >= p.Nb) {
                 if (held >= 0) { ptx::mbar_arrive(ptx::smem_u32(a_empty + held)); held = -1; }
                 continue;
diff --git a/hyperpose_b200/csrc/engine.cu b/hyperpose_b200/csrc/engine.cu
--- a/hyperpose_b200/csrc/engine.cu
+++ b/hyperpose_b200/csrc/engine.cu
@@ -732,11 +732,13 @@
     CUtensorMap tmap_a, tmap_b;
     CUtensorMap tmap_x;
     CUtensorMap tmap_o;
+    CUtensorMap tmap_c1, tmap_c2;
     void* d_w = nullptr;
     bool monotone_act = false;
     HaloParams hp;
     HaloItem halo_item = HaloItem::Narrow;
     bool halo_pool = false;
+    bool halo_chain = false;
     float* d_bias = nullptr;
     float* d_alpha = nullptr;
     float* d_mul = nullptr;
@@ -797,6 +799,7 @@
     bool stem3 = true;
     bool pool_fuse = true;
     bool dw1_fuse = true;
+    bool chain_fuse = true;
     bool dw_pair = true;
     bool dw_tma = true;
     int pifpaf_reserve_sms = 0;
@@ -955,6 +958,60 @@
     return HaloItem::Narrow;
 }
 
+bool dead_from(const hp_engine* e, size_t from, const PackOp& c, bool* rewritten)
+{
+    const int C = c.type == OP_CONV ? (int)c.groups * (int)c.cout_g : (int)c.cout_g;
+    *rewritten = false;
+    for (size_t k = from; k < e->ops.size() && !*rewritten; ++k) {
+        const PackOp& q = e->ops[k].po;
+        if (reads_buffer(q, c.out_buf)) return false;
+        if (q.type != OP_IM2COL3 && q.type != OP_PIFPAF_HEAD && q.type != OP_PPN_HEAD && q.out_mode != OUT_F32_NCHW_SPLIT && q.out_buf == c.out_buf) {
+            const int qc = q.type == OP_CONV ? (int)q.groups * (int)q.cout_g : (int)q.cout_g;
+            if (q.out_ch_off <= c.out_ch_off && (int)q.out_ch_off + qc >= (int)c.out_ch_off + C) *rewritten = true; else return false;
+        }
+    }
+    return true;
+}
+
+void fuse_chain(hp_engine* e, size_t i, const float* blob)
+{
+    EngOp& c = e->ops[i]; EngOp& d = e->ops[i + 1]; EngOp& o = e->ops[i + 2];
+    const HaloParams& h = c.plan.hp;
+    if (c.launch != Launch::Halo || c.plan.halo_item != HaloItem::Wide || c.plan.halo_pool || !h.tma_store || h.box_bytes < 2 * 128 * 128 ||
+        h.cout_g != h.cout_g_pad || h.groups * h.cout_g != 256)
+        return;
+    auto plain_1x1 = [](const EngOp& q) {
+        return q.launch == Launch::Conv && q.po.type == OP_CONV && q.po.R == 1 && q.po.S == 1 && !q.po.im2col_input && !q.po.res_mode &&
+               !q.plan.prm.post_w;
+    };
+    const PackOp &dp = d.po, &op = o.po;
+    if (!plain_1x1(d) || dp.out_mode != OUT_F16_NHWC || dp.groups != 2 || dp.cin_g != 128 || dp.cout_g != 128 || d.plan.prm.BN != 128 ||
+        dp.in_buf != c.po.out_buf || dp.in_ch_off != c.po.out_ch_off)
+        return;
+    if (!plain_1x1(o) || op.groups != 1 || op.cin_g != 256 || o.plan.prm.BN != 64 || o.plan.prm.cout_g_pad != 64 || op.in_buf != dp.out_buf ||
+        op.in_ch_off != dp.out_ch_off || (op.out_mode == OUT_F16_NHWC && op.out_buf == c.po.in_buf))
+        return;
+    const float* w = blob + op.w_off;
+    const int cout = (int)op.cout_g;
+    auto any = [&](int row, int c0) { for (int k = c0; k < c0 + 128; ++k) if (w[(size_t)row * 256 + k] != 0.f) return true; return false; };
+    int split = 0;
+    while (split < cout && !any(split, 128)) ++split;
+    for (int r = split; r < cout; ++r)
+        if (any(r, 0)) return;
+    bool rw_c = false, rw_d = false;
+    if (!dead_from(e, i + 2, c.po, &rw_c) || !dead_from(e, i + 3, dp, &rw_d) || !rw_c || !rw_d) return;
+    HaloParams& hh = c.plan.hp;
+    hh.c1_bias = d.plan.d_bias; hh.c1_alpha = d.plan.d_alpha;
+    hh.c2_bias = o.plan.d_bias; hh.c2_alpha = o.plan.d_alpha;
+    hh.c2_split = split; hh.c2_cout = cout;
+    const ConvParams& q = o.plan.prm;
+    hh.c2_mode = q.out_mode; hh.c2_out = q.out; hh.c2_out2 = q.out2;
+    hh.c2_out_ld = q.out_ld; hh.c2_out_ch_off = q.out_ch_off; hh.c2_plane_split = q.split;
+    c.plan.tmap_c1 = d.plan.tmap_b;
+    c.plan.tmap_c2 = o.plan.tmap_b;
+    c.plan.halo_chain = true;
+}
+
 int build_conv_plan(hp_engine* e, EngOp& op, const float* blob)
 {
     const PackOp& po = op.po;
@@ -1130,10 +1187,13 @@
     }
     return nullptr;
 }
-const void* halo_kernel(int BN, HaloItem item, bool pool)
+const void* halo_kernel(int BN, HaloItem item, bool pool, bool chain)
 {
     using I = HaloItem;
-    if (item == I::Wide) return BN == 128 && !pool ? (const void*)conv_halo_kernel<128, false, I::Wide> : nullptr;
+    if (item == I::Wide) {
+        if (BN != 128 || pool) return nullptr;
+        return chain ? (const void*)conv_halo_kernel<128, false, I::Wide, true> : (const void*)conv_halo_kernel<128, false, I::Wide>;
+    }
     if (item == I::PingPong) {
         if (BN == 64) return pool ? (const void*)conv_halo_kernel<64, true, I::PingPong> : (const void*)conv_halo_kernel<64, false, I::PingPong>;
         if (BN == 128) return pool ? (const void*)conv_halo_kernel<128, true, I::PingPong> : (const void*)conv_halo_kernel<128, false, I::PingPong>;
@@ -1177,7 +1237,7 @@
     else                          launch_pdl(dwconv3_tma_kernel<1, 1>, grid, DWT_THREADS, op.dwt_smem, st, op.tmap_dw, p);
 }
 
-int launch_conv(hp_engine* e, EngOp& op, int N, cudaStream_t st, bool u8_input)
+int launch_conv(hp_engine* e, EngOp& op, int N, cudaStream_t st, bool u8_input, bool chain = false)
 {
     ConvPlan& pl = op.plan;
     ConvParams p = pl.prm;
@@ -1191,8 +1251,8 @@
         const long items = ((long)N * h.tiles_x * h.tiles_y + tiles - 1) / tiles * h.groups * (h.cout_g_pad / p.BN);
         cudaLaunchAttribute at[1];
         const cudaLaunchConfig_t cfg = pdl_config((int)std::min<long>(e->num_sms - e->reserve_sms, items), CONV_THREADS, pl.smem, st, at);
-        void* args[] = { (void*)&pl.tmap_x, (void*)&pl.tmap_b, (void*)&pl.tmap_o, (void*)&h };
-        HP_CUDA_TRY(cudaLaunchKernelExC(&cfg, halo_kernel(p.BN, pl.halo_item, pl.halo_pool), args));
+        void* args[] = { (void*)&pl.tmap_x, (void*)&pl.tmap_b, (void*)&pl.tmap_o, (void*)&h, (void*)&pl.tmap_c1, (void*)&pl.tmap_c2 };
+        HP_CUDA_TRY(cudaLaunchKernelExC(&cfg, halo_kernel(p.BN, pl.halo_item, pl.halo_pool, pl.halo_chain && chain), args));
         return HP_OK;
     }
     p.m_tiles = (int)(((size_t)N * p.H * p.W + CONV_BLOCK_M - 1) / CONV_BLOCK_M);
@@ -1300,10 +1360,15 @@
     }
     tl_use_pdl = e->use_pdl;
     const uint8_t* frames = e->cur_frames ? e->cur_frames : e->d_frames;
+    int chain_end = -1;
     for (int oi = first; oi <= last; ++oi) {
         EngOp& op = e->ops[oi];
         const PackOp& po = op.po;
         const int K = (int)po.R, stride = po.stride ? (int)po.stride : 1;
+        if (oi <= chain_end) {
+            if (prof) cudaEventRecord(evset[oi + 1], st);
+            continue;
+        }
         switch (op.launch) {
         case Launch::None:
             break;
@@ -1322,9 +1387,15 @@
 #undef HP_IM2COL
             break;
         }
-        case Launch::Conv: case Launch::ConvStem: case Launch::Halo:
+        case Launch::Conv: case Launch::ConvStem:
             launch_conv(e, op, N, st, u8_input);
             break;
+        case Launch::Halo: {
+            const bool chain = op.plan.halo_chain && oi + 2 <= last;
+            launch_conv(e, op, N, st, u8_input, chain);
+            if (chain) chain_end = oi + 2;
+            break;
+        }
         case Launch::DwTma:
             launch_dw_tma(e, op, nullptr, N, st);
             break;
@@ -1562,6 +1633,7 @@
     opt.stem3 = !getenv("HPB_NO_STEM3");
     opt.pool_fuse = !getenv("HPB_NO_POOL_FUSE");
     opt.dw1_fuse = !getenv("HPB_NO_DW1_FUSE");
+    opt.chain_fuse = !getenv("HPB_NO_CHAIN_FUSE");
     opt.dw_pair = !getenv("HPB_NO_DW_DUAL");
     opt.dw_tma = !getenv("HPB_NO_DW_TMA");
     const char* rs = getenv("HPB_PIFPAF_RESERVE_SMS");
@@ -1736,16 +1808,8 @@
             if (cp.R != 1 || cp.S != 1 || cp.cin_g != cp.cout_g || cp.BN != cp.cout_g || (int)d.po.out_ch_off != cp.in_ch_off) continue;
         }
         if (c.po.res_mode && d.po.out_buf == c.po.res_buf) continue;
-        bool safe = true, rewritten = false;
-        for (size_t k = i + 2; k < e->ops.size() && safe && !rewritten; ++k) {
-            const PackOp& q = e->ops[k].po;
-            if (reads_buffer(q, c.po.out_buf)) safe = false;
-            else if (q.type != OP_IM2COL3 && q.type != OP_PIFPAF_HEAD && q.type != OP_PPN_HEAD && q.out_mode != OUT_F32_NCHW_SPLIT && q.out_buf == c.po.out_buf) {
-                const int qc = q.type == OP_CONV ? (int)q.groups * (int)q.cout_g : (int)q.cout_g;
-                if (q.out_ch_off <= c.po.out_ch_off && (int)q.out_ch_off + qc >= (int)c.po.out_ch_off + Ctot) rewritten = true; else safe = false;
-            }
-        }
-        if (!safe) continue;
+        bool rewritten = false;
+        if (!dead_from(e, i + 2, c.po, &rewritten)) continue;
         const EngBuffer& ob = e->bufs[d.po.out_buf];
         if ((int)d.po.out_ch_off + Ctot > ob.channels) continue;
         c.plan.prm.out = ob.d; c.plan.prm.out_ld = ob.channels; c.plan.prm.out_ch_off = (int)d.po.out_ch_off;
@@ -1753,6 +1817,7 @@
         d.launch = Launch::None;
         if (!rewritten) e->bufs[c.po.out_buf].fused_away = true;
     }
+    for (size_t i = 0; opt.chain_fuse && i + 2 < e->ops.size(); ++i) fuse_chain(e, i, blob.data());
     for (EngOp& c : e->ops) {
         if (c.launch != Launch::Conv && c.launch != Launch::ConvStem) continue;
         if (int rc = set_conv_tma_store(e, c)) return fail(rc);
@@ -1799,13 +1864,17 @@
     for (const EngOp& o : e->ops) {
         if ((o.po.type == OP_CONV || o.po.type == OP_DWCONV || o.po.type == OP_MAXPOOL2) && o.launch != Launch::None) ++launches;
         e->step_kernels += kernels_launched(o.launch, true);
+        if (o.launch == Launch::Halo && o.plan.halo_chain) {
+            launches -= 2;
+            e->step_kernels -= 2;
+        }
     }
     const double per_launch = launches ? e->flops_per_frame * e->max_batch / launches : 0.0;
     e->use_pdl = dtype == HP_DTYPE_F16 && launches > 0 && per_launch < 10e9;
     for (const EngOp& o : e->ops) {
         if (o.po.type != OP_CONV) continue;
         if (o.launch == Launch::Halo &&
-            cudaFuncSetAttribute(halo_kernel(o.plan.prm.BN, o.plan.halo_item, o.plan.halo_pool), cudaFuncAttributeMaxDynamicSharedMemorySize, (int)max_smem) != cudaSuccess) {
+            cudaFuncSetAttribute(halo_kernel(o.plan.prm.BN, o.plan.halo_item, o.plan.halo_pool, o.plan.halo_chain), cudaFuncAttributeMaxDynamicSharedMemorySize, (int)max_smem) != cudaSuccess) {
             set_error("engine: cannot opt in to %zu bytes of dynamic shared memory (halo)", max_smem);
             return fail(HP_ERR_CUDA);
         }
@@ -2204,6 +2273,14 @@
     return HP_OK;
 }
 
+int hp_engine_debug_op_chained(const hp_engine* e, int op, int* chained)
+{
+    if (!e || op < 0 || op >= (int)e->ops.size() || !chained) { set_error("hp_engine_debug_op_chained: bad argument"); return HP_ERR_ARG; }
+    const EngOp& o = e->ops[op];
+    *chained = o.launch == Launch::Halo && o.plan.halo_chain ? 1 : 0;
+    return HP_OK;
+}
+
 int hp_engine_debug_op_conv_epilogue(const hp_engine* e, int op, int* tma_store)
 {
     if (!e || op < 0 || op >= (int)e->ops.size() || !tma_store) { set_error("hp_engine_debug_op_conv_epilogue: bad argument"); return HP_ERR_ARG; }
diff --git a/include/hyperpose_b200.h b/include/hyperpose_b200.h
--- a/include/hyperpose_b200.h
+++ b/include/hyperpose_b200.h
@@ -131,6 +131,7 @@
 int hp_engine_debug_op_kernel(const hp_engine* e, int op, char* name, int cap);
 int hp_engine_debug_op_epilogue(const hp_engine* e, int op, int* tma_store);
 int hp_engine_debug_op_conv_epilogue(const hp_engine* e, int op, int* tma_store);
+int hp_engine_debug_op_chained(const hp_engine* e, int op, int* chained);
 int hp_engine_debug_uses_pdl(const hp_engine* e, int* pdl);
 
 int hp_engine_set_output_override(hp_engine* e, const float* d_conf, const float* d_paf);
```

Result: faster. 1158 (median of 6 runs) (+2.4%).
